# 2InfinityN6eyond/AbsoluteTrack

Measured on AMD Instinct MI355X. Metric: hand-frames/sec, higher is better.
Workload: dtype f32 (backbone products as two fp16 pieces per operand, fp32 accumulation); 1 GPU; 4 fisheye cameras x 2 hands per frame, 2 views per hand, 96x96 crops, known-skeleton path, full hot path (resample+backbone+head+FK) + all-gather of records; frames_per_gpu=1024, src_image=480x636 u8 x 4 cameras, parallelism=frame-shard x1, world=1, backend=none (single process), outputs_finite=True

## Files before the change

### absolutetrack_amd/csrc/conv_w4.hip

```cpp
#include "ut_kernels.h"
#include "ut_conv_dev.h"

namespace ut {
namespace {

constexpr int W4_WPIX = 288;
constexpr int W4_MI = 9;
constexpr int W4_NLOAD = 9;
constexpr int W4_NSTG = 5;
constexpr int W4_DIST = 2;
constexpr int W4_NSET = W4_DIST + 1;
constexpr unsigned W4_HOOB = 0x80000000u;
static_assert(9 % W4_NSET == 0, "the register sets of the weight fragments line up across slices");
constexpr int w4_cap(int pixels, int wi, int hi) { return ((pixels / (wi * hi)) * (hi + 1) * (wi + 1) + 2 * (wi + 2) + 15) / 16 * 16; }

template <int WI, int HI, int SCH, int WPX, bool S2 = false>
__global__ __launch_bounds__(256, 1) void conv_w4_kernel(ConvLaunch p, int tiles_n, int n_tiles) {
  extern __shared__ __attribute__((aligned(16))) char smem[];
  constexpr int MI = W4_MI, PW = WI + 1, PH = HI + 1, HW = WI * HI;
  static_assert(!S2 || (SCH == 32 && WPX == 1), "phase planes: two 16-channel planes per buffer, four 32-channel blocks per tile");
  constexpr int BM = W4_WPIX * WPX;
  constexpr int NCB = 4 / WPX, BN = 32 * NCB;
  constexpr int NG = SCH / 4, NHG = NG / 2;
  constexpr int KS = 9 * SCH / 16;
  constexpr int NBUF = SCH == 32 ? 2 : 3;
  constexpr int AHEAD = NBUF - 1;
  constexpr int RP = 256 / NG;
  constexpr int CAP = w4_cap(BM, WI, HI);
  constexpr int GSTRIDE = CAP * 16;
  constexpr int STAGE = NG * GSTRIDE;
  constexpr int SLOT = NBUF * STAGE;
  constexpr int EPI = SLOT + 16;
  static_assert(BM % HW == 0, "a tile is a whole number of maps: every tile has the same padded layout");
  static_assert(BM * NG == W4_NLOAD * 256 && KS % W4_NSET == 0 && (SCH == 32 || SCH == 16) && (WPX == 1 || WPX == 2), "shape");
  static_assert((NG - 2) * GSTRIDE + (2 * PW + 2) * 16 < 65536, "fragment reads: everything but the lane's base fits the immediate offset");

  const int tid = threadIdx.x;
  const int lane = tid & 63;
  const int wave = __builtin_amdgcn_readfirstlane(tid >> 6);
  const int wm = WPX == 1 ? 0 : wave >> 1;
  const int wco = WPX == 1 ? wave : wave & 1;
  const int fr = lane & 31, fh = lane >> 5;

  const int M = p.n_img * HW;
  const int n_slices = (!S2 && p.k_cin > 0 ? p.k_cin : p.cin) / (S2 ? 16 : SCH);
  const int n_chunks = p.k_pad / 32;

  const __amdgpu_buffer_rsrc_t a_rsrc = __builtin_amdgcn_make_buffer_rsrc(
      const_cast<float*>(p.in), 0, (int)((size_t)M * (S2 ? 4 : 1) * p.cin * sizeof(float)), 0x00020000);
  const __amdgpu_buffer_rsrc_t w_rsrc = __builtin_amdgcn_make_buffer_rsrc(
      const_cast<void*>(p.w_split), 0, (int)((size_t)(p.cout_pad / 32) * n_chunks * 4096), 0x00020000);
  const __amdgpu_buffer_rsrc_t r_rsrc = __builtin_amdgcn_make_buffer_rsrc(
      const_cast<float*>(p.res ? p.res : p.bias), 0, p.res ? (int)((size_t)M * p.cout_store * sizeof(float)) : 0, 0x00020000);
  const __amdgpu_buffer_rsrc_t o_rsrc =
      __builtin_amdgcn_make_buffer_rsrc(p.out, 0, (int)((size_t)M * p.cout_store * sizeof(float)), 0x00020000);
  const __amdgpu_buffer_rsrc_t q_rsrc = __builtin_amdgcn_make_buffer_rsrc(p.tile_counter, 0, 4, 0x00020000);

  float x_scale = 1.f, x_unscale = 1.f;
  if (p.in_max) {
    bool ok, adapted;
    split_act_scale(p.in_max, p.in_obs, p.split_adaptive, x_scale, x_unscale, ok, adapted);
    split_scale_report(ok, adapted, p.status, p.adapt_count);
  }
  const float tot_unscale = p.split_unscale * x_unscale;
  const float floor_v = p.relu ? 0.f : -__builtin_huge_valf();
  const unsigned row_b = (unsigned)p.cout_store * 4u;

  const int grid = gridDim.x;
  int slot = blockIdx.x;
  if ((grid & 7) == 0) slot = (blockIdx.x & 7) * (grid >> 3) + (blockIdx.x >> 3);

  unsigned h_wa[W4_NLOAD], pb[MI];
#pragma unroll
  for (int j = 0; j < W4_NLOAD; ++j) {
    const int k = RP * j + tid / NG, img = k / HW, rem = k - img * HW, y = rem / WI, x = rem - y * WI;
    h_wa[j] = (unsigned)((PW + 1 + img * (PH * PW) + y * PW + x) * 16 + ((tid % NG) >> 1) * GSTRIDE + (tid & 1) * 8);
  }
#pragma unroll
  for (int i = 0; i < MI; ++i) {
    const int k = wm * W4_WPIX + 32 * i + fr, img = k / HW, rem = k - img * HW, y = rem / WI, x = rem - y * WI;
    pb[i] = (unsigned)((img * (PH * PW) + y * PW + x) * 16 + fh * GSTRIDE);
  }
  const unsigned h_step = (unsigned)(RP * p.cin) * 4u;
#define W4_H_BASE(TILE) ((unsigned)((((TILE) / tiles_n) * BM + tid / NG) * p.cin + 4 * (tid % NG)) * 4u)
  unsigned h_in[S2 ? W4_NLOAD : 1], po_a = 0, po_b = 0, pb1[S2 ? MI : 1];
  if constexpr (S2) {
#pragma unroll
    for (int j = 0; j < W4_NLOAD; ++j) {
      const int k = RP * j + tid / NG, img = k / HW, rem = k - img * HW, y = rem / WI, x = rem - y * WI;
      h_in[j] = (unsigned)(((img * 2 * HI + 2 * y) * 2 * WI + 2 * x) * p.cin + 4 * (tid & 3)) * 4u;
    }
    const bool second = (tid & 4) != 0;
    po_a = second ? 0u : (unsigned)((2 * WI + 1) * p.cin) * 4u;
    po_b = second ? (unsigned)(2 * WI * p.cin) * 4u : (unsigned)p.cin * 4u;
#pragma unroll
    for (int i = 0; i < MI; ++i) pb1[i] = pb[i] + (unsigned)STAGE;
  }
#define W4S_BASE(TILE) ((unsigned)(((TILE) / tiles_n) * (BM * 4)) * (unsigned)p.cin * 4u)

  f32x16 acc[MI];
  u32x4 xp[MI][2];
  u32x4 wf[W4_NSET][2];
  float4 stg[S2 ? W4_NLOAD : W4_NSTG];
  const unsigned w_lane = (unsigned)lane * 16u;

#define W4_READ_X(I, PC, S, TAP, BASE)                                                               \
  xp[I][PC] = *reinterpret_cast<const u32x4*>(smem + (BASE)[I] + (unsigned)(((PC) * NHG + (SCH == 32 ? 2 * (S) : 0)) * GSTRIDE + (((TAP) / 3) * PW + (TAP) % 3) * 16));
#define W4_LOAD_W(SET, PL, CH, S, WROW)                                                              \
  {                                                                                                  \
    const unsigned so_ = (WROW) + (unsigned)((wco * n_chunks + (CH)) * 4096 + ((S) * 2 + (PL)) * 1024); \
    wf[SET][PL] = __builtin_bit_cast(u32x4, __builtin_amdgcn_raw_buffer_load_b128(w_rsrc, w_lane, so_, 0)); \
  }
#define W4S_PLANE(Q) ((0x190 >> (Q)) & 1)
#define W4S_TAPP(Q) ((int)((0x414344310ull >> (4 * (Q))) & 15))
#define W4S_TAPO(Q) ((int)((0x715348620ull >> (4 * (Q))) & 15))
#define W4S_BASEOF(Q) ((Q) >= 5 ? pb1 : pb)
#define W4_TAP(Q) (SCH == 32 ? (Q) >> 1 : (Q))
#define W4_CHUNK(SL, Q) (SCH == 32 ? (SL) * 9 + ((Q) >> 1) : ((SL) >> 1) * 9 + (Q))
#define W4_HALF(SL, Q) (SCH == 32 ? (Q) & 1 : (SL) & 1)
#define W4_MFMA(WSET, N)                                                                             \
  {                                                                                                  \
    constexpr int pr_ = (N) / MI, i_ = (N) % MI;                                                     \
    constexpr int wp_ = pr_ == 1 ? 1 : 0, xq_ = pr_ == 0 ? 1 : 0;       \
    acc[i_] = __builtin_amdgcn_mfma_f32_32x32x16_f16(__builtin_bit_cast(f16x8, xp[i_][xq_]),         \
                                                     __builtin_bit_cast(f16x8, wf[WSET][wp_]), acc[i_], 0, 0, 0);  \
  }
#define W4_PIN() { __builtin_amdgcn_sched_barrier(0); asm volatile("" ::: "memory"); __builtin_amdgcn_sched_barrier(0); }
#define W4_ROW_OFF(I, R) ((unsigned)((I) * 32 + 8 * ((R) >> 2) + ((R) & 3)) * row_bs)
#define W4_SPLIT_STORE(V, WA)                                                                        \
  {                                                                                                  \
    unsigned a0_, b0_, a1_, b1_;                                                                     \
    split_pair_scaled((V).x, (V).y, x_scale, a0_, b0_);                                              \
    split_pair_scaled((V).z, (V).w, x_scale, a1_, b1_);                                              \
    *reinterpret_cast<u32x2*>(smem + (WA)) = u32x2{a0_, a1_};                                        \
    *reinterpret_cast<u32x2*>(smem + (WA) + NHG * GSTRIDE) = u32x2{b0_, b1_};                        \
  }

  int tile = slot;
  int next_tile = 0;
  int cur_buf = 0;
  unsigned out_bits = 0;
  const unsigned slot_addr = (unsigned)(unsigned long)(lds_char*)smem + (unsigned)SLOT;

  for (int k = tid; k < NBUF * STAGE / 16; k += 256) *reinterpret_cast<u32x4*>(smem + k * 16) = u32x4{0, 0, 0, 0};
  __syncthreads();
  unsigned h_base = S2 ? 0u : W4_H_BASE(tile);
  unsigned w_row = (unsigned)((tile % tiles_n) * NCB) * (unsigned)n_chunks * 4096u;
  unsigned w_row_next = w_row;
  if constexpr (!S2) {
#pragma unroll
    for (int a = 0; a < AHEAD; ++a)
#pragma unroll
      for (int j = 0; j < W4_NLOAD; ++j) {
        const float4 v = __builtin_bit_cast(float4, __builtin_amdgcn_raw_buffer_load_b128(a_rsrc, h_base + (unsigned)j * h_step, (unsigned)(a * SCH * 4), 0));
        if (a == AHEAD - 1 && KS == 9 && j >= W4_NLOAD - 4) stg[j % W4_NSTG] = v;
        else W4_SPLIT_STORE(v, (unsigned)(a * STAGE) + h_wa[j])
      }
#pragma unroll
    for (int g = 0; g < W4_DIST; ++g) { W4_LOAD_W(g, 0, W4_CHUNK(0, g), W4_HALF(0, g), w_row) W4_LOAD_W(g, 1, W4_CHUNK(0, g), W4_HALF(0, g), w_row) }
  } else {
    const unsigned t0 = W4S_BASE(tile);
#pragma unroll
    for (int j = 0; j < W4_NLOAD; ++j) {
      const float4 v = __builtin_bit_cast(float4, __builtin_amdgcn_raw_buffer_load_b128(a_rsrc, h_in[j] + po_a + t0, 0, 0));
      W4_SPLIT_STORE(v, h_wa[j])
    }
#pragma unroll
    for (int j = 0; j < W4_NLOAD; ++j) {
      const float4 v = __builtin_bit_cast(float4, __builtin_amdgcn_raw_buffer_load_b128(a_rsrc, h_in[j] + po_b + t0, 0, 0));
      if (j == 0) W4_SPLIT_STORE(v, (unsigned)STAGE + h_wa[j])
      else stg[j] = v;
    }
#pragma unroll
    for (int g = 0; g < W4_DIST; ++g) { W4_LOAD_W(g, 0, W4S_TAPO(g), 0, w_row) W4_LOAD_W(g, 1, W4S_TAPO(g), 0, w_row) }
  }
  __syncthreads();
#pragma unroll
  for (int i = 0; i < MI; ++i) {
    W4_READ_X(i, 1, 0, 0, pb)
    if (i < MI - 1) { W4_READ_X(i, 0, 0, 0, pb) }
  }

#define W4_SLOT_BODY(N)                                                                              \
        {                                                                                            \
          if ((N) == 0 && q != KS - 1) { W4_READ_X(MI - 1, 0, W4_HALF(sl, q), W4_TAP(q), rb) }       \
          if ((N) >= 1 && (N) <= 9 && q1 < KS) { W4_READ_X(((N) + 8) % 9, 1, W4_HALF(sl, q1), W4_TAP(q1), rb) } \
          if ((N) >= 1 && (N) <= 9 && q1 == KS) { W4_READ_X(((N) + 8) % 9, 1, 0, 0, nb) }            \
          if ((N) >= 19 && (N) <= 26 && q1 < KS) { W4_READ_X(((N) + 8) % 9, 0, W4_HALF(sl, q1), W4_TAP(q1), rb) } \
          if ((N) >= 19 && (N) <= 26 && q1 == KS) { W4_READ_X(((N) + 8) % 9, 0, 0, 0, nb) }          \
          if (((N) == 10 || (N) == 11) && qd < KS) { W4_LOAD_W(qd % W4_NSET, (N) & 1, W4_CHUNK(sl, qd), W4_HALF(sl, qd), w_row) } \
          if (((N) == 10 || (N) == 11) && qd >= KS) { W4_LOAD_W(qd % W4_NSET, (N) & 1, W4_CHUNK(sl_after, qd - KS), W4_HALF(sl_after, qd - KS), row_after) } \
          if ((N) == 12 && q >= 4 && q < 4 + W4_NLOAD) { const float4 v_ = stg[(q + W4_NSTG - 4) % W4_NSTG]; split_pair_scaled(v_.x, v_.y, x_scale, cv0, cv1); } \
          if ((N) == 13 && q >= 4 && q < 4 + W4_NLOAD) {                                             \
            const float4 v_ = stg[(q + W4_NSTG - 4) % W4_NSTG];                                      \
            unsigned a1_, b1_;                                                                       \
            split_pair_scaled(v_.z, v_.w, x_scale, a1_, b1_);                                        \
            *reinterpret_cast<u32x2*>(smem + wbuf + h_wa[(q + 5) % 9]) = u32x2{cv0, a1_};            \
            *reinterpret_cast<u32x2*>(smem + wbuf + h_wa[(q + 5) % 9] + NHG * GSTRIDE) = u32x2{cv1, b1_}; \
          }                                                                                          \
          if (KS == 9 && (N) == 12 && q < 4) { const float4 v_ = stg[q % W4_NSTG]; split_pair_scaled(v_.x, v_.y, x_scale, cv0, cv1); } \
          if (KS == 9 && (N) == 13 && q < 4) {       \
            const float4 v_ = stg[q % W4_NSTG];                                                      \
            unsigned a1_, b1_;                                                                       \
            split_pair_scaled(v_.z, v_.w, x_scale, a1_, b1_);                                        \
            *reinterpret_cast<u32x2*>(smem + pbuf + h_wa[q + 5]) = u32x2{cv0, a1_};                  \
            *reinterpret_cast<u32x2*>(smem + pbuf + h_wa[q + 5] + NHG * GSTRIDE) = u32x2{cv1, b1_};  \
          }                                                                                          \
          if ((N) == 14 && q < W4_NLOAD)                                                             \
            stg[q % W4_NSTG] = __builtin_bit_cast(float4, __builtin_amdgcn_raw_buffer_load_b128(a_rsrc, h_base + (unsigned)q * h_step, f_soff, 0)); \
          if ((N) == 16 && q == KS / 2 && sl == 0 && tid == 0) *reinterpret_cast<int*>(smem + SLOT) = grid + ticket; \
          W4_PIN();                                                                                  \
          W4_MFMA(ws, N);                                                                            \
          W4_PIN();                                                                                  \
        }
#define W4_SLICE()                                                                                   \
      _Pragma("clang loop unroll(full)") for (int q = 0; q < KS; ++q) {                              \
        const int ws = q % W4_NSET;                                                                  \
        unsigned cv0 = 0, cv1 = 0;      \
         \
        const int q1 = q + 1, qd = q + W4_DIST;                                                      \
        if (q == KS - 1) {                                                                           \
                                       \
          W4_READ_X(MI - 1, 0, W4_HALF(sl, KS - 1), 8, rb)                                           \
          asm volatile("s_waitcnt lgkmcnt(0)" ::: "memory");                                         \
          __builtin_amdgcn_s_barrier();                                                              \
          asm volatile("" ::: "memory");                                                             \
          if (sl == 0) {                                                                             \
            next_tile = slot_read(slot_addr);                                                        \
            w_row_next = (unsigned)((next_tile % tiles_n) * NCB) * (unsigned)n_chunks * 4096u;       \
          }                                                                                          \
        }                                                                                            \
        W4_SLOT_BODY(0) W4_SLOT_BODY(1) W4_SLOT_BODY(2) W4_SLOT_BODY(3) W4_SLOT_BODY(4) W4_SLOT_BODY(5) W4_SLOT_BODY(6) W4_SLOT_BODY(7) W4_SLOT_BODY(8) \
        W4_SLOT_BODY(9) W4_SLOT_BODY(10) W4_SLOT_BODY(11) W4_SLOT_BODY(12) W4_SLOT_BODY(13) W4_SLOT_BODY(14) W4_SLOT_BODY(15) W4_SLOT_BODY(16) W4_SLOT_BODY(17) \
        W4_SLOT_BODY(18) W4_SLOT_BODY(19) W4_SLOT_BODY(20) W4_SLOT_BODY(21) W4_SLOT_BODY(22) W4_SLOT_BODY(23) W4_SLOT_BODY(24) W4_SLOT_BODY(25) W4_SLOT_BODY(26) \
      }

#define W4S_CV_N(Q) ((Q) == 4 ? 3 : (Q) == 8 ? 1 : 2)
#define W4S_CV_J(Q, NN) ((Q) < 4 ? 2 * (Q) + 1 + (NN) : (Q) == 4 ? (NN) : (Q) < 8 ? 2 * (Q) - 7 + (NN) : 0)
#define W4S_CV_DST(Q) (((Q) < 4 || (Q) == 8) ? (unsigned)STAGE : 0u)
#define W4S_LD_N(Q) ((Q) == 0 ? 3 : (Q) == 4 ? 1 : 2)
#define W4S_LD_J(Q, NN) ((Q) == 0 ? (NN) : (Q) < 4 ? 2 * (Q) + 1 + (NN) : (Q) == 4 ? 0 : 2 * (Q) - 9 + (NN))
#define W4S_SLOT_BODY(N)                                                                             \
        {                                                                                            \
          if ((N) == 0) { W4_READ_X(MI - 1, 0, W4S_PLANE(q), W4S_TAPP(q), W4S_BASEOF(q)) }          \
          if ((N) == 9 && (q == 4 || q == 8)) {                                                      \
                                         \
            asm volatile("s_waitcnt lgkmcnt(0)" ::: "memory");                                       \
            __builtin_amdgcn_s_barrier();                                                            \
            asm volatile("" ::: "memory");                                                           \
            if (q == 8 && sl == 0) {                                                                 \
              next_tile = slot_read(slot_addr);                                                      \
              w_row_next = (unsigned)((next_tile % tiles_n) * NCB) * (unsigned)n_chunks * 4096u;     \
            }                                                                                        \
          }                                                                                          \
          if ((N) >= 1 && (N) <= 9 && q != 4 && q != 8) { W4_READ_X(((N) + 8) % 9, 1, W4S_PLANE(q1), W4S_TAPP(q1), W4S_BASEOF(q1)) } \
          if ((N) >= 10 && (N) <= 18 && (q == 4 || q == 8)) { W4_READ_X(((N) + 8) % 9, 1, W4S_PLANE(q1), W4S_TAPP(q1), W4S_BASEOF(q1)) } \
          if ((N) >= 19 && (N) <= 26) { W4_READ_X(((N) + 8) % 9, 0, W4S_PLANE(q1), W4S_TAPP(q1), W4S_BASEOF(q1)) } \
          if (((N) == 10 || (N) == 11) && qd < 9) { W4_LOAD_W(qd % W4_NSET, (N) & 1, (sl >> 1) * 9 + W4S_TAPO(qd), sl & 1, w_row) } \
          if (((N) == 10 || (N) == 11) && qd >= 9) { W4_LOAD_W(qd % W4_NSET, (N) & 1, (sl_after >> 1) * 9 + W4S_TAPO(qd - 9), sl_after & 1, row_after) } \
           \
          if ((N) >= 10 && (N) <= 21 && ((N) - 10) / 4 < W4S_CV_N(q)) {                              \
            const float4 v_ = stg[W4S_CV_J(q, ((N) - 10) / 4) % 9];                                  \
            constexpr int part_ = ((N) - 10) & 3;                                                    \
            if (part_ == 0 || part_ == 2) {                                                          \
              const f16x2 h_ = __builtin_bit_cast(f16x2, __builtin_amdgcn_cvt_pkrtz((part_ ? v_.z : v_.x) * x_scale, (part_ ? v_.w : v_.y) * x_scale)); \
              (part_ ? cvh1 : cvh0) = __builtin_bit_cast(unsigned, h_);                              \
              cvf = (float)h_[0];                                                                    \
            } else {                                                                                 \
              const f16x2 h_ = __builtin_bit_cast(f16x2, part_ == 1 ? cvh0 : cvh1);                  \
              const float ra_ = __builtin_fmaf(part_ == 1 ? v_.x : v_.z, x_scale, -cvf);             \
              const float rb_ = __builtin_fmaf(part_ == 1 ? v_.y : v_.w, x_scale, -(float)h_[1]);    \
              const unsigned p_ = __builtin_bit_cast(unsigned, __builtin_amdgcn_cvt_pkrtz(ra_, rb_)); \
              if (part_ == 1) cvp0 = p_;                                                             \
              else {                                                                                 \
                *reinterpret_cast<u32x2*>(smem + W4S_CV_DST(q) + h_wa[W4S_CV_J(q, ((N) - 10) / 4) % 9]) = u32x2{cvh0, cvh1}; \
                *reinterpret_cast<u32x2*>(smem + W4S_CV_DST(q) + h_wa[W4S_CV_J(q, ((N) - 10) / 4) % 9] + NHG * GSTRIDE) = u32x2{cvp0, p_}; \
              }                                                                                      \
            }                                                                                        \
          }                                                                                          \
          if ((N) >= 22 && (N) <= 24 && (N) - 22 < W4S_LD_N(q))                                      \
            stg[W4S_LD_J(q, (N) - 22) % 9] = __builtin_bit_cast(float4, __builtin_amdgcn_raw_buffer_load_b128(    \
                a_rsrc, h_in[W4S_LD_J(q, (N) - 22) % 9] + (q < 4 ? hb_a : hb_b), f_soff, 0));        \
          if ((N) == 16 && q == 1 && sl == 0 && tid == 0) *reinterpret_cast<int*>(smem + SLOT) = grid + ticket; \
          W4_PIN();                                                                                  \
          W4_MFMA(ws, N);                                                                            \
          W4_PIN();                                                                                  \
        }
#define W4S_SLICE()                                                                                  \
      _Pragma("clang loop unroll(full)") for (int q = 0; q < 9; ++q) {                               \
        const int ws = q % W4_NSET;                                                                  \
        unsigned cvh0 = 0, cvh1 = 0, cvp0 = 0;                       \
        float cvf = 0.f;                                                                             \
        const int q1 = (q + 1) % 9, qd = q + W4_DIST;                                                \
        W4S_SLOT_BODY(0) W4S_SLOT_BODY(1) W4S_SLOT_BODY(2) W4S_SLOT_BODY(3) W4S_SLOT_BODY(4) W4S_SLOT_BODY(5) W4S_SLOT_BODY(6) W4S_SLOT_BODY(7) W4S_SLOT_BODY(8) \
        W4S_SLOT_BODY(9) W4S_SLOT_BODY(10) W4S_SLOT_BODY(11) W4S_SLOT_BODY(12) W4S_SLOT_BODY(13) W4S_SLOT_BODY(14) W4S_SLOT_BODY(15) W4S_SLOT_BODY(16) W4S_SLOT_BODY(17) \
        W4S_SLOT_BODY(18) W4S_SLOT_BODY(19) W4S_SLOT_BODY(20) W4S_SLOT_BODY(21) W4S_SLOT_BODY(22) W4S_SLOT_BODY(23) W4S_SLOT_BODY(24) W4S_SLOT_BODY(25) W4S_SLOT_BODY(26) \
      }

  for (;;) {
    int ticket = 0;
    if (tid == 0) ticket = __builtin_amdgcn_raw_ptr_buffer_atomic_add_i32(1, q_rsrc, 0, 0, 0);
#pragma unroll
    for (int i = 0; i < MI; ++i)
#pragma unroll
      for (int e = 0; e < 16; ++e) acc[i][e] = 0.f;

    const float4 bb4 = *reinterpret_cast<const float4*>(p.bias + (tile % tiles_n) * BN + wco * 32 + 4 * (lane & 7));
    if constexpr (S2) {
      for (int sl = 0; sl < n_slices; ++sl) {
        const bool last_slice = sl == n_slices - 1;
        const unsigned f_soff = last_slice ? 0u : (unsigned)(sl + 1) * 64u;
        const unsigned f_tb = W4S_BASE(last_slice ? next_tile : tile);
        const unsigned hb_a = po_a + f_tb, hb_b = po_b + f_tb;
        const int sl_after = last_slice ? 0 : sl + 1;
        const unsigned row_after = last_slice ? w_row_next : w_row;
        W4S_SLICE()
      }
    } else
    for (int sl = 0; sl < n_slices; ++sl) {
      const bool last_slice = sl == n_slices - 1;
      const int b1 = cur_buf + 1 == NBUF ? 0 : cur_buf + 1, b2 = b1 + 1 == NBUF ? 0 : b1 + 1;
      unsigned rbuf = (unsigned)__builtin_amdgcn_readfirstlane(cur_buf * STAGE), nbuf = (unsigned)__builtin_amdgcn_readfirstlane(b1 * STAGE);
      unsigned wbuf = (unsigned)__builtin_amdgcn_readfirstlane((NBUF == 2 ? b1 : b2) * STAGE), pbuf = nbuf;
      asm volatile("" : "+s"(rbuf), "+s"(nbuf), "+s"(wbuf), "+s"(pbuf));
      const int f_sl = sl + AHEAD < n_slices ? sl + AHEAD : sl + AHEAD - n_slices;
      if (sl + AHEAD == n_slices) h_base = W4_H_BASE(next_tile);
      const unsigned f_soff = (unsigned)f_sl * (SCH * 4);
      const int sl_after = last_slice ? 0 : sl + 1;
      const unsigned row_after = last_slice ? w_row_next : w_row;
      unsigned rb[MI], nb[MI];
#pragma unroll
      for (int i = 0; i < MI; ++i) { rb[i] = pb[i] + rbuf; nb[i] = pb[i] + nbuf; }
      W4_SLICE()
      cur_buf = b1;
    }
    {
      const int tm = tile / tiles_n, tn = tile - tm * tiles_n;
      const bool ragged = tm * BM + BM > M;
      const int ch = tn * BN + wco * 32 + fr;
      const float bb = p.bias[ch];
      const unsigned base = ch < p.cout_store ? (unsigned)((tm * BM + wm * W4_WPIX + 4 * fh) * p.cout_store + ch) * 4u : W4_HOOB;
      const unsigned keep_n = base != W4_HOOB ? 0x7FFFFFFFu : 0u;
      if (!ragged) {
        unsigned row_bs = (unsigned)__builtin_amdgcn_readfirstlane((int)row_b);
        asm volatile("" : "+s"(row_bs));
        const int ch4 = tn * BN + wco * 32 + 4 * (lane & 7);
        const unsigned base4 = ch4 < p.cout_store ? (unsigned)((tm * BM + wm * W4_WPIX + (lane >> 3)) * p.cout_store + ch4) * 4u : W4_HOOB;
        const unsigned keep4 = base4 != W4_HOOB ? 0x7FFFFFFFu : 0u;
        float4 rr[S2 ? 1 : 6][4];
        if constexpr (!S2) {
#pragma unroll
          for (int i = 0; i < 5; ++i)
#pragma unroll
            for (int t = 0; t < 4; ++t)
              rr[i][t] = __builtin_bit_cast(float4, __builtin_amdgcn_raw_buffer_load_b128(r_rsrc, base4, (unsigned)(32 * i + 8 * t) * row_bs, 0));
        }
        char* const ex = smem + EPI + wave * 4096;
#define W4_EX_WRITE(H)                                                                               \
        _Pragma("unroll") for (int r = 0; r < 8; ++r)                                                \
          *reinterpret_cast<float*>(ex + ((H) & 1) * 2048 + (8 * (r >> 2) + 4 * fh + (r & 3)) * 128 + fr * 4) = acc[(H) >> 1][8 * ((H) & 1) + r];
        W4_EX_WRITE(0)
#pragma unroll
        for (int h = 0; h < 2 * MI; ++h) {
          const int i = h >> 1;
          if (!S2 && (h & 1) == 0 && i + 5 < MI) {
#pragma unroll
            for (int t = 0; t < 4; ++t)
              rr[(i + 5) % 6][t] = __builtin_bit_cast(float4, __builtin_amdgcn_raw_buffer_load_b128(r_rsrc, base4, (unsigned)(32 * (i + 5) + 8 * t) * row_bs, 0));
          }
          if (h + 1 < 2 * MI) { W4_EX_WRITE(h + 1) }
#pragma unroll
          for (int t2 = 0; t2 < 2; ++t2) {
            const int t = 2 * (h & 1) + t2;
            const float4 a = *reinterpret_cast<const float4*>(ex + (h & 1) * 2048 + (8 * t2 + (lane >> 3)) * 128 + (lane & 7) * 16);
            const float4 res = S2 ? float4{0.f, 0.f, 0.f, 0.f} : rr[S2 ? 0 : i % 6][t];
            u32x4 o;
            o.x = __float_as_uint(fmaxf(fmaf(a.x, tot_unscale, bb4.x + res.x), floor_v));
            o.y = __float_as_uint(fmaxf(fmaf(a.y, tot_unscale, bb4.y + res.y), floor_v));
            o.z = __float_as_uint(fmaxf(fmaf(a.z, tot_unscale, bb4.z + res.z), floor_v));
            o.w = __float_as_uint(fmaxf(fmaf(a.w, tot_unscale, bb4.w + res.w), floor_v));
            unsigned mk;
            asm volatile("v_max3_u32 %0, %2, %3, %4\n\tv_max_u32 %0, %0, %5\n\tv_and_b32 %0, %0, %6\n\tv_max_u32 %1, %1, %0"
                         : "=&v"(mk), "+v"(out_bits) : "v"(o.x), "v"(o.y), "v"(o.z), "v"(o.w), "v"(keep4));
            __builtin_amdgcn_raw_buffer_store_b128(o, o_rsrc, base4, (unsigned)(32 * i + 8 * t) * row_bs, 0);
          }
        }
#undef W4_EX_WRITE
      } else {
#pragma unroll
        for (int i = 0; i < MI; ++i) {
          float r1[16];
          unsigned off = base + (unsigned)(i * 32) * row_b;
#pragma unroll
          for (int r = 0; r < 16; ++r) {
            r1[r] = __uint_as_float(__builtin_amdgcn_raw_buffer_load_b32(r_rsrc, off, 0, 0));
            off += ((r & 3) == 3 ? 5u : 1u) * row_b;
          }
          off = base + (unsigned)(i * 32) * row_b;
#pragma unroll
          for (int r = 0; r < 16; ++r) {
            const unsigned o = __float_as_uint(fmaxf(fmaf(acc[i][r], tot_unscale, bb + r1[r]), floor_v));
            const int pix = wm * W4_WPIX + i * 32 + 8 * (r >> 2) + 4 * fh + (r & 3);
            out_bits = max(out_bits, o & (tm * BM + pix < M ? keep_n : 0u));
            __builtin_amdgcn_raw_buffer_store_b32(o, o_rsrc, off, 0, 0);
            off += ((r & 3) == 3 ? 5u : 1u) * row_b;
          }
        }
      }
    }
    if ((unsigned)next_tile >= (unsigned)n_tiles) break;
    tile = next_tile;
    w_row = w_row_next;
  }
  if (p.out_max) publish_abs_max(p.out_max, out_bits);
#undef W4_H_BASE
#undef W4_READ_X
#undef W4_LOAD_W
#undef W4_TAP
#undef W4_CHUNK
#undef W4_HALF
#undef W4_MFMA
#undef W4_PIN
#undef W4_ROW_OFF
#undef W4_SPLIT_STORE
#undef W4_SLOT_BODY
#undef W4_SLICE
#undef W4S_PLANE
#undef W4S_TAPP
#undef W4S_TAPO
#undef W4S_BASEOF
#undef W4S_BASE
#undef W4S_CV_N
#undef W4S_CV_J
#undef W4S_CV_DST
#undef W4S_LD_N
#undef W4S_LD_J
#undef W4S_SLOT_BODY
#undef W4S_SLICE
}

template <int WI, int HI, int SCH, int WPX, bool S2 = false>
hipError_t launch_w4_cfg(const ConvLaunch& c, hipStream_t s) {
  constexpr int BM = W4_WPIX * WPX, BN = 128 / WPX;
  const long M = (long)c.n_img * c.Ho * c.Wo;
  const int tiles_m = (int)((M + BM - 1) / BM), tiles_n = c.cout_store / BN;
  const int n_tiles = tiles_m * tiles_n;
  constexpr int lds = (SCH == 32 ? 2 : 3) * (SCH / 4) * w4_cap(BM, WI, HI) * 16 + 16 + 4 * 4096;
  return launch_with_lds<&conv_w4_kernel<WI, HI, SCH, WPX, S2>>(c.device, lds, persistent_grid(c.num_cu, n_tiles), 256, s, c, tiles_n, n_tiles);
}

}

W4Form conv_w4_form(const ConvLaunch& c) {
  const bool common = c.w_split && c.split_unscale > 0.f && c.ksize == 3 && c.pad == 1 && c.cslice == 32 &&
                      c.cin % 32 == 0 && c.cout_pad >= c.cout_store && !c.out_nchw && c.splits == 0 &&
                      c.k_pad == 9 * c.cin && c.tile_counter && c.num_cu > 0 &&
                      offsets_fit_32(c.n_img, c.H, c.W, c.cin) && offsets_fit_32(c.n_img, c.Ho, c.Wo, c.cout_store);
  if (!common) return W4_NONE;
  if (c.stride == 2)
    return c.cin >= 64  && c.cout_store % 128 == 0 && c.H == 2 * c.Ho && c.W == 2 * c.Wo && !c.res &&
           ((c.Wo == 12 && c.Ho == 12) || (c.Wo == 6 && c.Ho == 6)) ? W4_STRIDE2 : W4_NONE;
  if (c.stride != 1 || c.cin < 64 || c.H != c.Ho || c.W != c.Wo) return W4_NONE;
  if (c.k_cin != 0 && (c.k_cin % 32 != 0 || c.k_cin < 64 || c.k_cin > c.cin)) return W4_NONE;
  if (c.cout_store % 128 == 0) return (c.W == 12 && c.H == 12) || (c.W == 6 && c.H == 6) ? W4_TILES128 : W4_NONE;
  return c.cout_store == 64 && c.W == 24 && c.H == 24 ? W4_MAP24 : W4_NONE;
}

hipError_t launch_conv_w4(const ConvLaunch& c, hipStream_t s) {
  const W4Form form = conv_w4_form(c);
  if (form == W4_NONE) return hipErrorInvalidValue;
  if (form == W4_STRIDE2) return c.Wo == 12 ? launch_w4_cfg<12, 12, 32, 1, true>(c, s) : launch_w4_cfg<6, 6, 32, 1, true>(c, s);
  if (form == W4_MAP24) return launch_w4_cfg<24, 24, 16, 2>(c, s);
  return c.W == 12 ? launch_w4_cfg<12, 12, 32, 1>(c, s) : launch_w4_cfg<6, 6, 32, 1>(c, s);
}

}
```

### absolutetrack_amd/csrc/ut_api.hip

```cpp
#include "../../include/umetrack_hip.h"
#include "../../include/umetrack_hip_fit.h"
#include "../../include/umetrack_hip_info.h"
#include "../../include/umetrack_hip_scale.h"
#include "../../include/umetrack_hip_triangulate.h"
#include "../../include/umetrack_hip_views.h"

#include <math.h>
#include <stdio.h>
#include <stdlib.h>
#include <string.h>

#include <cmath>
#include <initializer_list>
#include <mutex>
#include <string>
#include <utility>
#include <vector>

#include "ut_kernels.h"
#include "ut_weights.h"

namespace {

thread_local std::string g_create_error;

struct ConvW : ut::ConvGeom {
  float* w = nullptr;
  float* w_frag = nullptr;
  void* w_split = nullptr;
  float split_unscale = 0.f;
  float wsum_rows = 0.f;
  float bias_max = 0.f;
  float* bias = nullptr;
  int k_cin = 0;
};

struct Block {
  ConvW conv1, conv2, ds;
  bool has_ds = false;
};

struct Regressor {
  Block blocks[2];
  Block blocks_split[2];
  float* w_out = nullptr;
  float* b_out = nullptr;
  int c = 0, d = 0;
};

struct ProfEvent { hipEvent_t a, b; double flops;   int kind = 0;
};

}

constexpr int kDefaultChunk = 4096;
constexpr int kMaxChunk = 7281;

struct ut_context {
  int device = 0;
  int num_cu = 256;
  std::string err;
  std::vector<void*> allocs;
  float* stem_w = nullptr; float* stem_b = nullptr;
  Block bb[12];
  ConvW proj, fus0, fus1, fus2, tmp[3];
  float *skel_w = nullptr, *skel_b = nullptr, *skel_scale = nullptr, *skel_shift = nullptr;
  Regressor reg_k, reg_u;
  int chunk = kDefaultChunk;
  size_t ws_crops = 0;
  float *bufX = nullptr, *bufH = nullptr, *bufY = nullptr, *bufD = nullptr;
  size_t crops_ws_floats = 0;
  float* crops_ws = nullptr;
  size_t wsb_crops = 0;
  float *bufL2 = nullptr, *bufP = nullptr, *bufQ = nullptr, *bufBH = nullptr, *bufBD = nullptr;
  size_t ws_samples = 0;
  ut::HeadBuffers hb{};
  size_t ws_skel = 0;
  int slots_cap = 0, slots_used = 0;
  float *mem = nullptr, *prev_ext = nullptr;
  unsigned* counters = nullptr;
  int counter_next = 0;
  unsigned* calib = nullptr;
  unsigned* adapt_count = nullptr;
  int scale_mode = UT_SPLIT_SCALE_CALIBRATED;
  bool calibrated = false;
  bool head_calibrated = false;
  bool calibrating = false;
  unsigned word_gen = 0;
  bool block_fusion = true;
  int resident_weights = 1;
  bool call_split = false;
  int* status = nullptr;
  int* status_host = nullptr;
  int* slot_seen = nullptr;
  int check_mode = UT_CHECK_SYNC;
  int lanes = 1;
  hipStream_t lane_stream[2] = {nullptr, nullptr};
  hipEvent_t ev_fork = nullptr, ev_join[2] = {nullptr, nullptr};
  int conv_arith = UT_CONV_FP32;
  bool latency_mode = false;
  float* splitk_ws = nullptr;
  size_t splitk_floats = 0;
  float* zero_bias = nullptr;
  bool profiling = false;
  std::vector<ProfEvent> prof;
};

namespace {

int fail(ut_handle h, int code, const char* what, hipError_t e = hipSuccess) {
  char buf[512];
  if (e != hipSuccess) snprintf(buf, sizeof buf, "%s: %s", what, hipGetErrorString(e));
  else snprintf(buf, sizeof buf, "%s", what);
  if (h) h->err = buf; else g_create_error = buf;
  return code;
}

#define HIPCHK(h, x)                                            \
  do {                                                          \
    hipError_t e_ = (x);                                        \
    if (e_ != hipSuccess) return fail(h, UT_E_HIP, #x, e_);     \
  } while (0)

struct DeviceScope {
  int prev = -1;
  bool switched = false;
  hipError_t err = hipSuccess;
  explicit DeviceScope(int dev) {
    if (dev < 0) return;
    err = hipGetDevice(&prev);
    if (err == hipSuccess && prev != dev) {
      err = hipSetDevice(dev);
      switched = err == hipSuccess;
    }
  }
  ~DeviceScope() { if (switched) (void)hipSetDevice(prev); }
  DeviceScope(const DeviceScope&) = delete;
  DeviceScope& operator=(const DeviceScope&) = delete;
};
#define ON_DEVICE_IF(h)                                        \
  DeviceScope scope_((h) ? (h)->device : -1);                  \
  if ((h) && scope_.err != hipSuccess) return fail(h, UT_E_HIP, "hipSetDevice", scope_.err)
#define ON_DEVICE_OF(h)                 \
  DeviceScope scope_((h)->device);      \
  if (scope_.err != hipSuccess) return fail(h, UT_E_HIP, "hipSetDevice", scope_.err)

struct DevStatus { int* dev = nullptr; int* host = nullptr; };
std::mutex g_status_mutex;
DevStatus g_status[64];

int stateless_status(int* device_out, DevStatus* out) {
  int dev = 0;
  hipError_t e = hipGetDevice(&dev);
  if (e != hipSuccess) return fail(nullptr, UT_E_HIP, "hipGetDevice", e);
  if (dev < 0 || dev >= 64) return fail(nullptr, UT_E_INVALID, "device index beyond 63");
  std::lock_guard<std::mutex> lock(g_status_mutex);
  DevStatus& st = g_status[dev];
  if (!st.dev) {
    void *d = nullptr, *hst = nullptr;
    if ((e = hipMalloc(&d, 2 * sizeof(int))) != hipSuccess) return fail(nullptr, UT_E_HIP, "hipMalloc", e);
    if ((e = hipHostMalloc(&hst, 2 * sizeof(int), hipHostMallocDefault)) != hipSuccess) {
      (void)hipFree(d);
      return fail(nullptr, UT_E_HIP, "hipHostMalloc", e);
    }
    if ((e = hipMemset(d, 0, 2 * sizeof(int))) != hipSuccess) return fail(nullptr, UT_E_HIP, "hipMemset", e);
    st.dev = (int*)d; st.host = (int*)hst;
  }
  *device_out = dev;
  *out = st;
  return UT_OK;
}

const char* status_message(int bits) {
  if (bits & ut::UT_SPLIT_RANGE)
    return "range check: an activation entering a split-fp16 convolution is an infinity or a NaN, or lies beyond the calibrated range "
           "of its layer (32 x the calibration maximum; ut_calibrate_split with representative crops, UT_SPLIT_SCALE_DYNAMIC or "
           "UT_SPLIT_SCALE_CALIBRATED_ADAPTIVE)";
  if (bits & ut::UT_BAD_SRC_INDEX) return "index check: src_index outside [0, n_src_images)";
  if (bits & ut::UT_BAD_SAMPLE_RANGE) return "index check: sample_range rows must select 1 or 2 crops inside [0, n_crops]";
  if (bits & ut::UT_BAD_MEMORY_IDX) return "index check: memory_idx outside [0, n_slots)";
  if (bits & ut::UT_DUP_MEMORY_IDX) return "index check: memory_idx names one temporal slot twice";
  if (bits & ut::UT_BAD_HAND_IDX) return "index check: hand_idx must be 0 (left) or 1 (right)";
  return "index check: failed";
}

int check_status(ut_handle h, int* dev, int* host, hipStream_t s, const char* what) {
  HIPCHK(h, hipMemcpyAsync(host, dev, 2 * sizeof(int), hipMemcpyDeviceToHost, s));
  HIPCHK(h, hipStreamSynchronize(s));
  const int sticky = host[0];
  if (sticky) HIPCHK(h, hipMemsetAsync(dev, 0, sizeof(int), s));
  if (sticky & ut::UT_STATUS_ERRORS) {
    char buf[256];
    snprintf(buf, sizeof buf, "%s: %s", what, status_message(sticky));
    return fail(h, UT_E_INVALID, buf);
  }
  return UT_OK;
}

int upload_bytes(ut_handle h, const void* host, size_t bytes, void** dev) {
  void* d = nullptr;
  HIPCHK(h, hipMalloc(&d, bytes));
  h->allocs.push_back(d);
  HIPCHK(h, hipMemcpy(d, host, bytes, hipMemcpyHostToDevice));
  *dev = d;
  return UT_OK;
}

int upload(ut_handle h, const std::vector<float>& host, float** dev) {
  return upload_bytes(h, host.data(), host.size() * sizeof(float), (void**)dev);
}

int upload_conv(ut_handle h, ConvW& cw, const ut::PackedConv& pc) {
  static_cast<ut::ConvGeom&>(cw) = pc;
  cw.split_unscale = pc.split_unscale; cw.wsum_rows = pc.wsum_rows; cw.bias_max = pc.bias_max;
  int rc = upload(h, pc.wp, &cw.w);
  if (!rc && !pc.wfrag.empty()) rc = upload(h, pc.wfrag, &cw.w_frag);
  if (!rc && !pc.planes.empty()) rc = upload_bytes(h, pc.planes.data(), pc.planes.size() * sizeof(uint16_t), &cw.w_split);
  return rc ? rc : upload(h, pc.bp, &cw.bias);
}

int upload_block(ut_handle h, Block& b, const ut::FoldedBlock& fb, bool pw_ds = false) {
  int rc;
  const int cs = ut::round_up(fb.conv1.cout, 4);
  if ((rc = upload_conv(h, b.conv1, ut::pack_conv_host(fb.conv1, 3, fb.stride, cs)))) return rc;
  if ((rc = upload_conv(h, b.conv2, ut::pack_conv_host(fb.conv2, 3, 1, cs)))) return rc;
  b.has_ds = fb.has_ds;
  if (fb.has_ds && (rc = upload_conv(h, b.ds, ut::pack_conv_host(fb.ds, 1, fb.stride, cs, pw_ds)))) return rc;
  return UT_OK;
}

int upload_regressor(ut_handle h, Regressor& r, const ut::FoldedRegressor& fr) {
  r.c = fr.c; r.d = fr.d;
  int rc;
  for (int i = 0; i < 2; ++i)
    if ((rc = upload_block(h, r.blocks[i], fr.blocks[i])) || (rc = upload_block(h, r.blocks_split[i], fr.wide[i]))) return rc;
  for (int i = 0; i < 2; ++i) {
    r.blocks_split[i].conv1.k_cin = ut::round_up(fr.blocks[i].conv1.cin, 32);
    r.blocks_split[i].conv2.k_cin = ut::round_up(fr.blocks[i].conv2.cin, 32);
  }
  if ((rc = upload(h, fr.w_out, &r.w_out))) return rc;
  return upload(h, fr.b_out, &r.b_out);
}

int dev_alloc(ut_handle h, float** p, size_t n_floats) {
  void* d = nullptr;
  HIPCHK(h, hipMalloc(&d, n_floats * sizeof(float)));
  h->allocs.push_back(d);
  *p = (float*)d;
  return UT_OK;
}

void dev_free(ut_handle h, void* p) {
  if (!p) return;
  for (size_t i = 0; i < h->allocs.size(); ++i)
    if (h->allocs[i] == p) { h->allocs.erase(h->allocs.begin() + i); break; }
  (void)hipFree(p);
}

int regrow(ut_handle h, size_t* cap, size_t n, std::initializer_list<std::pair<float**, size_t>> bufs) {
  if (n <= *cap) return UT_OK;
  HIPCHK(h, hipDeviceSynchronize());
  for (auto& b : bufs) { dev_free(h, *b.first); *b.first = nullptr; }
  *cap = 0;
  int rc;
  for (auto& b : bufs)
    if ((rc = dev_alloc(h, b.first, n * b.second))) return rc;
  *cap = n;
  return UT_OK;
}

int ensure_backbone_ws(ut_handle h, int crops) {
  const size_t big = 48 * 48 * 32, small = 24 * 24 * 64;
  return regrow(h, &h->ws_crops, crops, {{&h->bufX, big}, {&h->bufH, big}, {&h->bufY, big}, {&h->bufD, small}});
}

constexpr int PHASE_B_MAX = 8192;

int ensure_phase_b_ws(ut_handle h, int crops) {
  const size_t l2 = 24 * 24 * 64, l3 = 12 * 12 * 128;
  return regrow(h, &h->wsb_crops, crops, {{&h->bufL2, l2}, {&h->bufP, l3}, {&h->bufQ, l3}, {&h->bufBH, l3}, {&h->bufBD, l3}});
}

int ensure_head_ws(ut_handle h, int samples, int n_skel) {
  ut::HeadBuffers& b = h->hb;
  const size_t r = 36 * ut::kRegSplitCh;
  int rc = regrow(h, &h->ws_samples, samples, {{&b.cat144, 36 * 144}, {&b.f108, 36 * 108}, {&b.f72a, 36 * 72}, {&b.f72b, 36 * 72},
                                                {&b.fused, 36 * 72}, {&b.t92a, 36 * 92}, {&b.t92b, 36 * 92}, {&b.regin, r},
                                                {&b.rega, r}, {&b.regb, r}});
  return rc ? rc : regrow(h, &h->ws_skel, n_skel, {{&b.skel, 36 * 4}});
}

int ensure_slots(ut_handle h, int slots, hipStream_t s) {
  if (slots <= h->slots_cap) return UT_OK;
  int cap = h->slots_cap ? h->slots_cap : 2;
  while (cap < slots) cap *= 2;
  float *nm = nullptr, *ne = nullptr, *seen = nullptr;
  int rc;
  if ((rc = dev_alloc(h, &nm, (size_t)cap * 36 * 18)) || (rc = dev_alloc(h, &ne, (size_t)cap * 16)) ||
      (rc = dev_alloc(h, &seen, (size_t)cap)))
    return rc;
  HIPCHK(h, hipMemsetAsync(nm, 0, (size_t)cap * 36 * 18 * sizeof(float), s));
  HIPCHK(h, hipMemsetAsync(ne, 0, (size_t)cap * 16 * sizeof(float), s));
  if (h->slots_cap) {
    HIPCHK(h, hipMemcpyAsync(nm, h->mem, (size_t)h->slots_cap * 36 * 18 * sizeof(float), hipMemcpyDeviceToDevice, s));
    HIPCHK(h, hipMemcpyAsync(ne, h->prev_ext, (size_t)h->slots_cap * 16 * sizeof(float), hipMemcpyDeviceToDevice, s));
    HIPCHK(h, hipStreamSynchronize(s));
    dev_free(h, h->mem);
    dev_free(h, h->prev_ext);
    dev_free(h, h->slot_seen);
  }
  h->mem = nm; h->prev_ext = ne; h->slot_seen = (int*)seen; h->slots_cap = cap;
  return UT_OK;
}

constexpr int kMaxCounters = 4096;
constexpr int kScaleTensors = 33;
static_assert(kScaleTensors < 63, "the adaptation counter is the last of the 64 words at ut_context::calib");
constexpr int kCalibHeadroom = 4;

int begin_call(ut_handle h, hipStream_t s) {
  h->counter_next = 0;
  ++h->word_gen;
  HIPCHK(h, ut::launch_zero_words(h->counters, 2 * kMaxCounters, s));
  return UT_OK;
}

int lease_words(ut_handle h, hipStream_t s, int n, bool* zeroed = nullptr) {
  const bool full = h->counter_next + n > kMaxCounters;
  if (zeroed) *zeroed = full;
  return full ? begin_call(h, s) : UT_OK;
}
int take_word(ut_handle h) { return h->counter_next++; }

struct ScaleRef { const unsigned* word = nullptr; const unsigned* obs = nullptr; int adaptive = 0; unsigned* adapt_count = nullptr; };
ScaleRef scale_for(ut_handle h, int tid, const unsigned* producer_word) {
  ScaleRef r;
  if (!h->call_split || h->latency_mode || tid < 0 || tid >= kScaleTensors) return r;
  if (h->calibrating || h->scale_mode == UT_SPLIT_SCALE_DYNAMIC) r.word = producer_word;
  else { r.word = h->calib + tid; r.obs = producer_word; }
  if (!h->calibrating && h->scale_mode == UT_SPLIT_SCALE_CALIBRATED_ADAPTIVE && r.obs) { r.adaptive = 1; r.adapt_count = h->adapt_count; }
  return r;
}
template <class Launch>
void set_scale(Launch& l, const ScaleRef& sr, int* status) {
  l.in_max = sr.word; l.in_obs = sr.obs; l.split_adaptive = sr.adaptive; l.adapt_count = sr.adapt_count; l.status = status;
}
template <class Launch>
int bracket_launch(ut_handle h, hipStream_t s, int in_tid, const unsigned* in_max, double flops, int kind, const char* what,
                   Launch launch) {
  if (h->calibrating && in_max && in_tid >= 0 && in_tid < kScaleTensors) HIPCHK(h, ut::launch_merge_max(h->calib + in_tid, in_max, s));
  ProfEvent pe{nullptr, nullptr, flops, kind};
  if (h->profiling) {
    HIPCHK(h, hipEventCreateWithFlags(&pe.a, hipEventDisableSystemFence));
    HIPCHK(h, hipEventCreateWithFlags(&pe.b, hipEventDisableSystemFence));
    HIPCHK(h, hipEventRecord(pe.a, s));
  }
  const hipError_t e = launch();
  if (e != hipSuccess) return fail(h, UT_E_HIP, what, e);
  if (h->profiling) {
    HIPCHK(h, hipEventRecord(pe.b, s));
    h->prof.push_back(pe);
  }
  return UT_OK;
}

int run_conv(ut_handle h, const ConvW& cw, const float* in, const float* res, float* out, int n_img, int H, int W,
             bool relu, bool nchw, hipStream_t s, const unsigned* in_max = nullptr, unsigned** out_max = nullptr, int in_tid = -1) {
  if (out_max) *out_max = nullptr;
  ut::ConvLaunch c{};
  c.in = in; c.w = cw.w; c.bias = cw.bias; c.res = res; c.out = out;
  c.n_img = n_img; c.H = H; c.W = W; c.cin = cw.cin_pad;
  c.Ho = (H + 2 * cw.pad - cw.ksize) / cw.stride + 1;
  c.Wo = (W + 2 * cw.pad - cw.ksize) / cw.stride + 1;
  c.cout_store = cw.cout_store; c.cout_pad = cw.cout_pad;
  c.k_total = cw.k_total; c.k_pad = cw.k_pad; c.cslice = cw.cslice;
  c.k_cin = h->block_fusion && cw.k_cin < cw.cin_pad ? cw.k_cin : 0;
  c.ksize = cw.ksize; c.stride = cw.stride; c.pad = cw.pad;
  c.relu = relu; c.out_nchw = nchw;
  c.device = h->device; c.num_cu = h->num_cu; c.no_resident = ut::kResidentKinds[h->resident_weights];
  bool zeroed = false;
  int rc = lease_words(h, s, 1, &zeroed);
  if (rc) return rc;
  if (zeroed) in_max = nullptr;
  const int word = take_word(h);
  c.tile_counter = h->counters + word;
  int splits = 1;
  if (h->latency_mode && !nchw && cw.cout_store % 4 == 0) {
    const long m = (long)n_img * c.Ho * c.Wo;
    const long tiles64 = ((m + 63) / 64) * ((cw.cout_store + 63) / 64);
    const int chunks = cw.k_pad / 32;
    for (int sp = 2; sp <= chunks / 6; ++sp)
      if (chunks % sp == 0 && tiles64 * sp <= (long)h->num_cu && (size_t)sp * m * cw.cout_store <= h->splitk_floats) splits = sp;
  }
  if (h->latency_mode) c.splits = 1;
  if (splits > 1) {
    ut::ConvLaunch part = c;
    part.bias = h->zero_bias; part.res = nullptr; part.relu = 0; part.out = h->splitk_ws; part.splits = splits;
    HIPCHK(h, ut::launch_conv_igemm(part, s));
    HIPCHK(h, ut::launch_splitk_finish(h->splitk_ws, splits, n_img * c.Ho * c.Wo, cw.cout_store, cw.bias, res, out,
                                       relu ? 1 : 0, s));
    return UT_OK;
  }
  const ScaleRef sr = scale_for(h, in_tid, in_max);
  c.w_split = sr.word ? cw.w_split : nullptr;
  c.split_unscale = cw.split_unscale;
  set_scale(c, sr, h->status);
  const ut::ConvKernel kernel = ut::choose_conv(c);
  const int kind = c.w_split && kernel != ut::CONV_IGEMM ? 1 : 0;
  if (kind) {
    c.out_max = h->counters + kMaxCounters + word;
    if (out_max) *out_max = c.out_max;
  }
  return bracket_launch(h, s, kind ? in_tid : -1, in_max, cw.flops_per_pixel * (double)n_img * c.Ho * c.Wo, kind,
                        ut::kConvKernelName[kernel], [&] { return ut::launch_conv_on(kernel, c, s); });
}

int run_pw(ut_handle h, std::initializer_list<const ConvW*> layers, std::initializer_list<bool> relus, const float* in, float* out,
           int n_img, int H, int W, bool nchw, hipStream_t s, bool* done) {
  *done = false;
  if (!h->block_fusion || h->latency_mode) return UT_OK;
  ut::PwLaunch c{};
  double flops = 0;
  const ConvW& first = **layers.begin();
  c.in = in; c.out = out; c.n_img = n_img; c.H = H; c.W = W; c.cin = first.cin_pad; c.stride = first.stride;
  c.Ho = (H - 1) / first.stride + 1; c.Wo = (W - 1) / first.stride + 1;
  c.out_nchw = nchw; c.num_cu = h->num_cu;
  auto relu = relus.begin();
  for (const ConvW* cw : layers) {
    if (cw->ksize != 1 || cw->pad != 0 || !cw->w_frag || (c.n_layers > 0 && cw->stride != 1)) return UT_OK;
    c.layer[c.n_layers++] = ut::PwLayer{cw->w_frag, cw->bias, cw->k_pad, cw->cout_store, cw->cout_pad, *relu++ ? 1 : 0};
    c.cout_store = cw->cout_store;
    flops += cw->flops_per_pixel * (double)n_img * c.Ho * c.Wo;
  }
  if (!ut::conv_pw_applicable(c)) return UT_OK;
  *done = true;
  return bracket_launch(h, s, -1, nullptr, flops, 0, "launch_conv_pw", [&] { return ut::launch_conv_pw(c, s); });
}

int run_block(ut_handle h, const Block& b, const float* x, float* tmp, float* dsbuf, float* y, int n_img, int H,
              int W, hipStream_t s, const unsigned* x_max = nullptr, unsigned** y_max = nullptr, int x_tid = -1, int mid_tid = -1) {
  int rc;
  if (y_max) *y_max = nullptr;
  bool zeroed = false;
  if ((rc = lease_words(h, s, 8, &zeroed))) return rc;
  if (zeroed) x_max = nullptr;
  const ScaleRef xs = scale_for(h, x_tid, x_max);
  if (h->block_fusion && xs.word && !b.has_ds && b.conv1.w_split && b.conv2.w_split && b.conv1.stride == 1 &&
      b.conv1.cin_pad == 32 && b.conv1.cout_store == 32 && b.conv2.cout_store == 32) {
    ut::BlockLaunch bl{};
    bl.in = x; bl.out = y; bl.w1_split = b.conv1.w_split; bl.w2_split = b.conv2.w_split;
    bl.unscale_w1 = b.conv1.split_unscale; bl.unscale_w2 = b.conv2.split_unscale;
    bl.bias1 = b.conv1.bias; bl.bias2 = b.conv2.bias;
    bl.wsum1 = b.conv1.wsum_rows; bl.bmax1 = b.conv1.bias_max;
    set_scale(bl, xs, h->status);
    bl.n_img = n_img; bl.H = H; bl.W = W; bl.device = h->device; bl.num_cu = h->num_cu;
    bl.tile_counter = h->counters + h->counter_next;
    if (ut::conv_block32_applicable(bl)) {
      bl.out_max = h->counters + kMaxCounters + take_word(h);
      const double flops = (b.conv1.flops_per_pixel + b.conv2.flops_per_pixel) * (double)n_img * H * W;
      if ((rc = bracket_launch(h, s, x_tid, x_max, flops, 1, "conv_block32", [&] { return ut::launch_conv_block32(bl, s); })))
        return rc;
      if (y_max) *y_max = bl.out_max;
      return UT_OK;
    }
  }
  if (h->block_fusion && xs.word && b.has_ds && b.conv1.w_split && b.ds.w_split && b.conv2.w_split &&
      b.conv1.stride == 2 && b.conv1.cin_pad == 32 && b.conv1.cout_store == 64 && b.ds.cout_store == 64 && dsbuf) {
    ut::Stride2Launch sl{};
    sl.in = x; sl.out1 = tmp; sl.out2 = dsbuf; sl.w1_split = b.conv1.w_split; sl.wd_split = b.ds.w_split;
    sl.unscale1 = b.conv1.split_unscale; sl.unscale_d = b.ds.split_unscale;
    sl.bias1 = b.conv1.bias; sl.bias_d = b.ds.bias;
    set_scale(sl, xs, h->status);
    sl.n_img = n_img; sl.H = H; sl.W = W; sl.device = h->device; sl.num_cu = h->num_cu;
    if (ut::conv_c32s2_applicable(sl)) {
      sl.out1_max = h->counters + kMaxCounters + take_word(h);
      const double flops = (b.conv1.flops_per_pixel + b.ds.flops_per_pixel) * (double)n_img * (H / 2) * (W / 2);
      if ((rc = bracket_launch(h, s, x_tid, x_max, flops, 1, "conv_c32s2", [&] { return ut::launch_conv_c32s2(sl, s); })))
        return rc;
      return run_conv(h, b.conv2, tmp, dsbuf, y, n_img, H / 2, W / 2, true, false, s, sl.out1_max, y_max, mid_tid);
    }
  }
  unsigned* tmp_max = nullptr;
  if ((rc = run_conv(h, b.conv1, x, nullptr, tmp, n_img, H, W, true, false, s, x_max, &tmp_max, x_tid))) return rc;
  const int Ho = (H + 2 - 3) / b.conv1.stride + 1, Wo = (W + 2 - 3) / b.conv1.stride + 1;
  const float* res = x;
  if (b.has_ds) {
    bool streamed = false;
    if ((rc = run_pw(h, {&b.ds}, {false}, x, dsbuf, n_img, H, W, false, s, &streamed))) return rc;
    if (!streamed && (rc = run_conv(h, b.ds, x, nullptr, dsbuf, n_img, H, W, false, false, s))) return rc;
    res = dsbuf;
  }
  return run_conv(h, b.conv2, tmp, res, y, n_img, Ho, Wo, true, false, s, tmp_max, y_max, mid_tid);
}

void prof_clear(ut_handle h) {
  for (auto& pe : h->prof) { (void)hipEventDestroy(pe.a); (void)hipEventDestroy(pe.b); }
  h->prof.clear();
}

int prof_reduce(ut_handle h, hipStream_t s, double ms[2], int64_t launches[2], double flops[2]) {
  h->profiling = false;
  HIPCHK(h, hipStreamSynchronize(s));
  for (int k = 0; k < 2; ++k) { ms[k] = 0; launches[k] = 0; flops[k] = 0; }
  for (auto& pe : h->prof) {
    float t = 0;
    HIPCHK(h, hipEventElapsedTime(&t, pe.a, pe.b));
    const int k = pe.kind ? 1 : 0;
    ms[k] += t; flops[k] += pe.flops; launches[k] += 1;
  }
  prof_clear(h);
  return UT_OK;
}

}

extern "C" {

size_t ut_weight_blob_floats(void) { return UT_WEIGHT_BLOB_FLOATS; }

const char* ut_last_error(ut_handle h) { return h ? h->err.c_str() : g_create_error.c_str(); }

int ut_canonical_backbone_weights(const float* blob, size_t n_floats, float* out, size_t out_floats, size_t* n_out) {
  if (!blob || !n_out) return fail(nullptr, UT_E_INVALID, "ut_canonical_backbone_weights: null argument");
  if (n_floats != UT_WEIGHT_BLOB_FLOATS) return fail(nullptr, UT_E_WEIGHTS, "ut_canonical_backbone_weights: weight blob has the wrong length");
  ut::FoldedNetwork net;
  if (!ut::fold_network(blob, n_floats, net)) return fail(nullptr, UT_E_WEIGHTS, "weight blob length does not match the architecture");
  const ut::FoldedBackbone& fbb = net.backbone;
  std::vector<const ut::Folded*> all = {&fbb.stem};
  for (const ut::FoldedBlock& b : fbb.fb) {
    all.push_back(&b.conv1); all.push_back(&b.conv2);
    if (b.has_ds) all.push_back(&b.ds);
  }
  all.push_back(&fbb.proj);
  size_t n = 0;
  for (const ut::Folded* f : all) n += f->w.size() + f->b.size();
  *n_out = n;
  if (!out) return UT_OK;
  if (out_floats < n) return fail(nullptr, UT_E_INVALID, "ut_canonical_backbone_weights: output too small");
  for (const ut::Folded* f : all) {
    memcpy(out, f->w.data(), f->w.size() * sizeof(float)); out += f->w.size();
    memcpy(out, f->b.data(), f->b.size() * sizeof(float)); out += f->b.size();
  }
  return UT_OK;
}

int ut_create(int device, const float* blob, size_t n_floats, ut_handle* out) {
  if (!blob || !out) return fail(nullptr, UT_E_INVALID, "ut_create: null argument");
  if (n_floats != UT_WEIGHT_BLOB_FLOATS) return fail(nullptr, UT_E_WEIGHTS, "ut_create: weight blob has the wrong length");
  ut::FoldedNetwork net;
  if (!ut::fold_network(blob, n_floats, net)) return fail(nullptr, UT_E_WEIGHTS, "weight blob length does not match the architecture");
  DeviceScope scope(device);
  if (scope.err != hipSuccess) return fail(nullptr, UT_E_HIP, "hipSetDevice", scope.err);
  ut_handle h = new ut_context();
  h->device = device;
  {
    int cus = 0;
    if (hipDeviceGetAttribute(&cus, hipDeviceAttributeMultiprocessorCount, device) == hipSuccess && cus > 0) h->num_cu = cus;
  }
  int rc = UT_OK;
  do {
    { float* cnt = nullptr; if ((rc = dev_alloc(h, &cnt, 2 * kMaxCounters + 64))) break; h->counters = (unsigned*)cnt;
      h->calib = h->counters + 2 * kMaxCounters;
      h->adapt_count = h->calib + 63;
      hipError_t e1 = hipMemset(h->calib, 0, 64 * sizeof(unsigned));
      if (e1 != hipSuccess) { rc = fail(h, UT_E_HIP, "calibration words", e1); break; } }
    { float* st = nullptr; if ((rc = dev_alloc(h, &st, 2))) break; h->status = (int*)st;
      hipError_t e2 = hipMemset(h->status, 0, 2 * sizeof(int));
      if (e2 == hipSuccess) e2 = hipHostMalloc((void**)&h->status_host, 2 * sizeof(int), hipHostMallocDefault);
      if (e2 != hipSuccess) { rc = fail(h, UT_E_HIP, "status words", e2); break; } }
    const ut::FoldedBackbone& fbb = net.backbone;
    if ((rc = upload(h, fbb.stem.w, &h->stem_w)) || (rc = upload(h, fbb.stem.b, &h->stem_b))) break;
    for (int b = 0; b < 12 && !rc; ++b) rc = upload_block(h, h->bb[b], fbb.fb[b], b == 10);
    if (rc) break;
    if ((rc = upload_conv(h, h->proj, ut::pack_conv_host(fbb.proj, 1, 1, 72, true)))) break;
    if ((rc = upload_conv(h, h->fus0, ut::pack_conv_host(net.fusion[0], 1, 1, 108, true))) ||
        (rc = upload_conv(h, h->fus1, ut::pack_conv_host(net.fusion[1], 1, 1, 72, true))) ||
        (rc = upload_conv(h, h->fus2, ut::pack_conv_host(net.fusion[2], 1, 1, 72, true)))) break;
    for (int i = 0; i < 3 && !rc; ++i) rc = upload_conv(h, h->tmp[i], ut::pack_conv_host(net.temporal[i], 1, 1, 92, true));
    if (rc) break;
    if ((rc = upload(h, net.skel_w, &h->skel_w)) || (rc = upload(h, net.skel_b, &h->skel_b)) ||
        (rc = upload(h, net.skel_scale, &h->skel_scale)) || (rc = upload(h, net.skel_shift, &h->skel_shift))) break;
    if ((rc = upload_regressor(h, h->reg_k, net.reg_k))) break;
    rc = upload_regressor(h, h->reg_u, net.reg_u);
  } while (0);
  if (rc) {
    g_create_error = h->err;
    ut_destroy(h);
    return rc;
  }
  *out = h;
  return UT_OK;
}

int ut_destroy(ut_handle h) {
  if (!h) return UT_OK;
  DeviceScope scope(h->device);
  (void)hipDeviceSynchronize();
  for (void* p : h->allocs) (void)hipFree(p);
  if (h->status_host) (void)hipHostFree(h->status_host);
  for (int i = 0; i < 2; ++i) {
    if (h->lane_stream[i]) (void)hipStreamDestroy(h->lane_stream[i]);
    if (h->ev_join[i]) (void)hipEventDestroy(h->ev_join[i]);
  }
  if (h->ev_fork) (void)hipEventDestroy(h->ev_fork);
  prof_clear(h);
  delete h;
  return UT_OK;
}

int ut_set_backbone_chunk(ut_handle h, int crops_per_pass) {
  if (!h || crops_per_pass < 0) return fail(h, UT_E_INVALID, "ut_set_backbone_chunk: bad argument");
  if (crops_per_pass > kMaxChunk) return fail(h, UT_E_INVALID, "ut_set_backbone_chunk: at most 7281 crops per pass (32-bit offsets)");
  h->chunk = crops_per_pass == 0 ? kDefaultChunk : crops_per_pass;
  return UT_OK;
}

int ut_reserve(ut_handle h, int max_crops, int max_samples, int max_slots) {
  if (!h) return UT_E_INVALID;
  ON_DEVICE_OF(h);
  int rc;
  int c = max_crops < h->chunk ? max_crops : h->chunk;
  if (c > 0 && (rc = ensure_backbone_ws(h, c))) return rc;
  int cb = max_crops < PHASE_B_MAX ? max_crops : PHASE_B_MAX;
  if (cb > 0 && (rc = ensure_phase_b_ws(h, cb))) return rc;
  if (max_samples > 0 && (rc = ensure_head_ws(h, max_samples, max_samples))) return rc;
  if (max_slots > 0 && (rc = ensure_slots(h, max_slots, 0))) return rc;
  if (max_crops > 0 && (rc = regrow(h, &h->crops_ws_floats, (size_t)max_crops * 96 * 96, {{&h->crops_ws, 1}}))) return rc;
  return UT_OK;
}

int ut_warp_crops(ut_handle h, const uint8_t* src, int n_src_images, int src_h, int src_w, const double* cam_params,
                  const double* crop_params, const int32_t* src_index, int n_crops, int remap_mode, float* out,
                  void* stream) {
  if (n_crops == 0) return UT_OK;
  if (!src || !cam_params || !crop_params || !src_index || !out || n_crops < 0 || src_h <= 0 || src_w <= 0 ||
      n_src_images <= 0 || (remap_mode != UT_REMAP_CV2_FIXED && remap_mode != UT_REMAP_FLOAT))
    return fail(h, UT_E_INVALID, "ut_warp_crops: bad argument");
  hipStream_t s = (hipStream_t)stream;
  int *st_dev = nullptr, *st_host = nullptr, mode = UT_CHECK_SYNC, dev = 0;
  if (h) { st_dev = h->status; st_host = h->status_host; mode = h->check_mode; dev = h->device; }
  else {
    DevStatus st;
    int rc = stateless_status(&dev, &st);
    if (rc) return rc;
    st_dev = st.dev; st_host = st.host;
  }
  DeviceScope scope(dev);
  if (scope.err != hipSuccess) return fail(h, UT_E_HIP, "hipSetDevice", scope.err);
  HIPCHK(h, ut::launch_warp(src, n_src_images, src_h, src_w, cam_params, crop_params, src_index, n_crops, remap_mode,
                            out, nullptr, st_dev, s));
  return mode == UT_CHECK_SYNC ? check_status(h, st_dev, st_host, s, "ut_warp_crops") : UT_OK;
}

extern "C" int ut_warp_map(const double* cam_params, const double* crop_params, const int32_t* src_index, int n_src_images,
                           int n_crops, float* out_map, void* stream) {
  if (n_crops == 0) return UT_OK;
  if (!cam_params || !crop_params || !src_index || !out_map || n_crops < 0 || n_src_images <= 0)
    return fail(nullptr, UT_E_INVALID, "ut_warp_map: bad argument");
  HIPCHK(nullptr, ut::launch_warp_map(cam_params, crop_params, src_index, n_src_images, n_crops, out_map, (hipStream_t)stream));
  return UT_OK;
}

static int run_stem(ut_handle h, const float* crops, const uint8_t* crops_u8, float* out, int n, hipStream_t st,
                    unsigned** out_max) {
  *out_max = nullptr;
  if (h->call_split && !h->latency_mode) {
    const int rc = lease_words(h, st, 1);
    if (rc) return rc;
    *out_max = h->counters + kMaxCounters + take_word(h);
  }
  if (crops_u8) HIPCHK(h, ut::launch_stem_u8(crops_u8, h->stem_w, h->stem_b, out, n, *out_max, st));
  else HIPCHK(h, ut::launch_stem(crops, h->stem_w, h->stem_b, out, n, *out_max, st));
  return UT_OK;
}

static int backbone_pass(ut_handle h, const float* crops, const uint8_t* crops_u8, float* feat, int c0, int n, int off,
                         int chunk, hipStream_t s) {
  int rc;
  const size_t a48 = (size_t)off * 48 * 48 * 32, a24 = (size_t)off * 24 * 24 * 64, a12 = (size_t)off * 12 * 12 * 128;
  if ((rc = lease_words(h, s, 256))) return rc;
  unsigned* l2_max = nullptr;
  const unsigned l2_gen = h->word_gen;
  for (int done = 0; done < n; done += chunk) {
    const int m = n - done < chunk ? n - done : chunk;
    const size_t first = (size_t)(c0 + done) * 96 * 96;
    unsigned* xm = nullptr;
    if ((rc = run_stem(h, crops ? crops + first : nullptr, crops_u8 ? crops_u8 + first : nullptr, h->bufX + a48, m, s, &xm))) return rc;
    float *x = h->bufX + a48, *y = h->bufY + a48;
    int hw = 48;
    for (int b = 0; b < 5; ++b) {
      float* dst = b == 4 ? h->bufL2 + a24 + (size_t)done * 24 * 24 * 64 : y;
      if ((rc = run_block(h, h->bb[b], x, h->bufH + a48, h->bufD + a24, dst, m, hw, hw, s, xm, &xm, 2 * b, 2 * b + 1))) return rc;
      hw = (hw + 2 - 3) / h->bb[b].conv1.stride + 1;
      float* t = x; x = y; y = t;
    }
    if (done == 0) l2_max = xm;
    else if (l2_max && xm) HIPCHK(h, ut::launch_merge_max(l2_max, xm, s));
    else l2_max = nullptr;
  }
  const float* x = h->bufL2 + a24;
  float *y = h->bufP + a12, *other = h->bufQ + a12;
  int hw = 24;
  unsigned* xm = l2_gen == h->word_gen ? l2_max : nullptr;
  for (int b = 5; b < 12; ++b) {
    if ((rc = run_block(h, h->bb[b], x, h->bufBH + a12, h->bufBD + a12, y, n, hw, hw, s, xm, &xm, 2 * b, 2 * b + 1))) return rc;
    hw = (hw + 2 - 3) / h->bb[b].conv1.stride + 1;
    x = y;
    float* t = y; y = other; other = t;
  }
  bool streamed = false;
  if ((rc = run_pw(h, {&h->proj}, {false}, x, feat + (size_t)c0 * 72 * 36, n, 6, 6, true, s, &streamed)) || streamed) return rc;
  return run_conv(h, h->proj, x, nullptr, feat + (size_t)c0 * 72 * 36, n, 6, 6, false, true, s);
}

static int run_backbone(ut_handle h, const float* crops, const uint8_t* crops_u8, int n_crops, float* feat, hipStream_t s) {
  int rc;
  const int chunk = n_crops < h->chunk ? n_crops : h->chunk;
  if ((rc = ensure_backbone_ws(h, chunk))) return rc;
  const int pass_b = n_crops < PHASE_B_MAX ? n_crops : PHASE_B_MAX;
  if ((rc = ensure_phase_b_ws(h, pass_b))) return rc;
  if ((rc = begin_call(h, s))) return rc;
  h->call_split = h->conv_arith == UT_CONV_SPLIT_F16_ALWAYS || (h->conv_arith == UT_CONV_SPLIT_F16 && n_crops >= 2 * h->num_cu);
  if (h->lanes == 2 && !h->profiling && n_crops <= chunk && n_crops <= pass_b && n_crops >= 1024) {
    if (!h->lane_stream[0]) {
      for (int i = 0; i < 2; ++i) {
        HIPCHK(h, hipStreamCreateWithFlags(&h->lane_stream[i], hipStreamNonBlocking));
        HIPCHK(h, hipEventCreateWithFlags(&h->ev_join[i], hipEventDisableTiming));
      }
      HIPCHK(h, hipEventCreateWithFlags(&h->ev_fork, hipEventDisableTiming));
    }
    HIPCHK(h, hipEventRecord(h->ev_fork, s));
    const int n0 = n_crops / 2;
    for (int i = 0; i < 2; ++i) {
      const int off = i ? n0 : 0, n = i ? n_crops - n0 : n0;
      HIPCHK(h, hipStreamWaitEvent(h->lane_stream[i], h->ev_fork, 0));
      if ((rc = backbone_pass(h, crops, crops_u8, feat, off, n, off, chunk, h->lane_stream[i]))) return rc;
      HIPCHK(h, hipEventRecord(h->ev_join[i], h->lane_stream[i]));
    }
    for (int i = 0; i < 2; ++i) HIPCHK(h, hipStreamWaitEvent(s, h->ev_join[i], 0));
    return UT_OK;
  }
  for (int base = 0; base < n_crops; base += pass_b) {
    const int nb = n_crops - base < pass_b ? n_crops - base : pass_b;
    if ((rc = backbone_pass(h, crops, crops_u8, feat, base, nb, 0, chunk, s))) return rc;
  }
  return UT_OK;
}

static int run_head(ut_handle h, const ut::HeadArgs& a, const float* skel, int n_skel, int mode, float* out_pose, float* out_raw,
                    hipStream_t s);

static int calibrate_head(ut_handle h, const float* feat, int n_crops, hipStream_t s) {
  const int S = n_crops / 2;
  int rc = ensure_head_ws(h, S, 1);
  if (rc) return rc;
  const size_t nf = (size_t)2 * S * 25 + 132 + (size_t)S * (648 + 16 + 60 + 64);
  const size_t off_i64 = (nf * 4 + 7) / 8 * 8, off_i32 = off_i64 + (size_t)4 * S * 8, off_u8 = off_i32 + (size_t)S * 4, total = off_u8 + S;
  std::vector<char> host(total, 0);
  float* f = reinterpret_cast<float*>(host.data());
  for (int c = 0; c < 2 * S; ++c) {
    float* k = f + (size_t)c * 9;
    k[0] = k[4] = 130.f; k[2] = k[5] = 47.5f; k[8] = 1.f;
    float* x = f + (size_t)2 * S * 9 + (size_t)c * 16;
    x[0] = x[5] = x[10] = x[15] = 1.f;
    if (c & 1) x[3] = 0.06f;
  }
  long long* i64 = reinterpret_cast<long long*>(host.data() + off_i64);
  for (int k = 0; k < S; ++k) { i64[2 * k] = 2 * k; i64[2 * k + 1] = 2 * k + 2; i64[2 * S + k] = k; i64[3 * S + k] = k & 1; }
  void* dv = nullptr;
  HIPCHK(h, hipMalloc(&dv, total));
  hipError_t e = hipMemcpyAsync(dv, host.data(), total, hipMemcpyHostToDevice, s);
  if (e == hipSuccess) e = hipStreamSynchronize(s);
  if (e != hipSuccess) { (void)hipFree(dv); return fail(h, UT_E_HIP, "calibration descriptors", e); }
  char* d = static_cast<char*>(dv);
  float* df = reinterpret_cast<float*>(d);
  ut::HeadArgs a{};
  a.feat = feat; a.intrinsics = df; a.extrinsics = df + (size_t)2 * S * 9;
  const float* skel = df + (size_t)2 * S * 25;
  a.mem = df + (size_t)2 * S * 25 + 132; a.prev_ext = a.mem + (size_t)S * 648;
  float* pose = a.prev_ext + (size_t)S * 16;
  float* raw = pose + (size_t)S * 60;
  a.sample_range = reinterpret_cast<const int64_t*>(d + off_i64); a.memory_idx = a.sample_range + 2 * S; a.hand_idx = a.memory_idx + S;
  a.slot_seen = reinterpret_cast<int*>(d + off_i32); a.use_memory = reinterpret_cast<const uint8_t*>(d + off_u8);
  a.n_samples = S; a.n_crops = 2 * S; a.n_slots = S; a.status = h->status; a.call_error_mask = 0;
  rc = begin_call(h, s);
  for (int mode = 0; mode < 2 && !rc; ++mode) rc = run_head(h, a, skel, 1, mode == 0 ? UT_MODE_KNOWN_SKELETON : UT_MODE_UNKNOWN_SKELETON, pose, raw, s);
  (void)hipStreamSynchronize(s);
  (void)hipFree(dv);
  return rc;
}

static int calibrate_split(ut_handle h, const float* crops, int n, hipStream_t s) {
  struct PinnedModes {
    ut_handle h;
    const int conv_arith, lanes;
    const bool profiling, block_fusion, latency_mode;
    explicit PinnedModes(ut_handle hh)
        : h(hh), conv_arith(hh->conv_arith), lanes(hh->lanes), profiling(hh->profiling), block_fusion(hh->block_fusion),
          latency_mode(hh->latency_mode) {
      h->conv_arith = UT_CONV_SPLIT_F16_ALWAYS; h->lanes = 1; h->profiling = false; h->latency_mode = false; h->calibrating = true;
    }
    ~PinnedModes() {
      h->conv_arith = conv_arith; h->lanes = lanes; h->profiling = profiling; h->block_fusion = block_fusion;
      h->latency_mode = latency_mode; h->calibrating = false;
    }
  };
  float* feat = nullptr;
  int rc = dev_alloc(h, &feat, (size_t)n * 72 * 36);
  if (rc) return rc;
  rc = [&]() -> int {
    PinnedModes pinned(h);
    int saved[2] = {0, 0}, r;
    HIPCHK(h, hipStreamSynchronize(s));
    HIPCHK(h, hipMemcpy(saved, h->status, sizeof saved, hipMemcpyDeviceToHost));
    h->calibrated = h->head_calibrated = false;
    HIPCHK(h, ut::launch_zero_words(h->calib, 64, s));
    for (int form = 0; form < 2; ++form) {
      h->block_fusion = form == 0;
      if ((r = run_backbone(h, crops, nullptr, n, feat, s))) return r;
    }
    const bool with_head = n >= 2;
    if (with_head && (r = calibrate_head(h, feat, n, s))) return r;
    HIPCHK(h, ut::launch_raise_words(h->calib, kScaleTensors, kCalibHeadroom, s));
    HIPCHK(h, hipStreamSynchronize(s));
    HIPCHK(h, hipMemcpy(h->status, saved, sizeof saved, hipMemcpyHostToDevice));
    h->calibrated = true;
    h->head_calibrated = with_head;
    return UT_OK;
  }();
  (void)hipStreamSynchronize(s);
  dev_free(h, feat);
  return rc;
}

constexpr int kBuiltinCalibCrops = 64;

static int calibrate_builtin(ut_handle h) {
  float* crops = nullptr;
  int rc = dev_alloc(h, &crops, (size_t)kBuiltinCalibCrops * 96 * 96);
  if (rc) return rc;
  hipError_t e = ut::launch_calibration_crops(crops, kBuiltinCalibCrops, 0);
  rc = e != hipSuccess ? fail(h, UT_E_HIP, "launch_calibration_crops", e) : calibrate_split(h, crops, kBuiltinCalibCrops, 0);
  (void)hipDeviceSynchronize();
  dev_free(h, crops);
  return rc;
}

int ut_calibrate_split(ut_handle h, const float* crops, int n_crops, void* stream) {
  if (!h) return UT_E_INVALID;
  if (n_crops < 0 || (n_crops > 0 && !crops)) return fail(h, UT_E_INVALID, "ut_calibrate_split: bad argument");
  ON_DEVICE_OF(h);
  return n_crops == 0 ? calibrate_builtin(h) : calibrate_split(h, crops, n_crops, (hipStream_t)stream);
}

int ut_set_split_scale(ut_handle h, int mode) {
  if (!h || (mode != UT_SPLIT_SCALE_CALIBRATED && mode != UT_SPLIT_SCALE_DYNAMIC && mode != UT_SPLIT_SCALE_CALIBRATED_ADAPTIVE))
    return fail(h, UT_E_INVALID, "ut_set_split_scale: bad argument");
  ON_DEVICE_OF(h);
  h->scale_mode = mode;
  if (mode != UT_SPLIT_SCALE_DYNAMIC && h->conv_arith != UT_CONV_FP32 && !h->calibrated) return calibrate_builtin(h);
  return UT_OK;
}

int ut_get_split_adaptations(ut_handle h, uint32_t* out, int reset, void* stream) {
  if (!h || !out) return fail(h, UT_E_INVALID, "ut_get_split_adaptations: null argument");
  ON_DEVICE_OF(h);
  hipStream_t s = (hipStream_t)stream;
  unsigned n = 0;
  HIPCHK(h, hipMemcpyAsync(&n, h->adapt_count, sizeof n, hipMemcpyDeviceToHost, s));
  HIPCHK(h, hipStreamSynchronize(s));
  *out = n;
  if (reset) {
    HIPCHK(h, ut::launch_zero_words(h->adapt_count, 1, s));
    HIPCHK(h, hipStreamSynchronize(s));
  }
  return UT_OK;
}

int ut_get_split_calibration(ut_handle h, float* out33) {
  if (!h || !out33) return fail(h, UT_E_INVALID, "ut_get_split_calibration: null argument");
  ON_DEVICE_OF(h);
  HIPCHK(h, hipDeviceSynchronize());
  HIPCHK(h, hipMemcpy(out33, h->calib, kScaleTensors * sizeof(float), hipMemcpyDeviceToHost));
  return h->calibrated ? UT_OK : 1;
}

int ut_backbone(ut_handle h, const float* crops, int n_crops, float* feat, void* stream) {
  if (!h) return UT_E_INVALID;
  if (n_crops == 0) return UT_OK;
  if (!crops || !feat || n_crops < 0) return fail(h, UT_E_INVALID, "ut_backbone: bad argument");
  ON_DEVICE_OF(h);
  return run_backbone(h, crops, nullptr, n_crops, feat, (hipStream_t)stream);
}

int ut_warp_backbone(ut_handle h, const uint8_t* src, int n_src_images, int src_h, int src_w, const double* cam_params,
                     const double* crop_params, const int32_t* src_index, int n_crops, int remap_mode, float* feat,
                     void* stream) {
  if (!h) return UT_E_INVALID;
  if (n_crops == 0) return UT_OK;
  if (!src || !cam_params || !crop_params || !src_index || !feat || n_crops < 0 || src_h <= 0 || src_w <= 0 ||
      n_src_images <= 0 || (remap_mode != UT_REMAP_CV2_FIXED && remap_mode != UT_REMAP_FLOAT))
    return fail(h, UT_E_INVALID, "ut_warp_backbone: bad argument");
  ON_DEVICE_OF(h);
  hipStream_t s = (hipStream_t)stream;
  const bool u8 = remap_mode == UT_REMAP_CV2_FIXED;
  int rc = regrow(h, &h->crops_ws_floats, (size_t)n_crops * 96 * 96 / (u8 ? sizeof(float) : 1), {{&h->crops_ws, 1}});
  if (rc) return rc;
  HIPCHK(h, ut::launch_warp(src, n_src_images, src_h, src_w, cam_params, crop_params, src_index, n_crops, remap_mode,
                            u8 ? nullptr : h->crops_ws, u8 ? (uint8_t*)h->crops_ws : nullptr, h->status, s));
  if (h->check_mode == UT_CHECK_SYNC && (rc = check_status(h, h->status, h->status_host, s, "ut_warp_backbone"))) return rc;
  return run_backbone(h, u8 ? nullptr : h->crops_ws, u8 ? (const uint8_t*)h->crops_ws : nullptr, n_crops, feat, s);
}

static int run_head(ut_handle h, const ut::HeadArgs& a, const float* skel, int n_skel, int mode, float* out_pose, float* out_raw,
                    hipStream_t s) {
  int rc;
  const ut::HeadBuffers& b = h->hb;
  const int S = a.n_samples;
  h->call_split = false;
  HIPCHK(h, ut::launch_ftl_in(a, b, h->block_fusion, s));
  bool chained = false;
  if ((rc = run_pw(h, {&h->fus0, &h->fus1, &h->fus2}, {true, true, false}, b.cat144, b.f72b, S, 6, 6, false, s, &chained))) return rc;
  if (!chained) {
    if ((rc = run_conv(h, h->fus0, b.cat144, nullptr, b.f108, S, 6, 6, true, false, s))) return rc;
    if ((rc = run_conv(h, h->fus1, b.f108, nullptr, b.f72a, S, 6, 6, true, false, s))) return rc;
    if ((rc = run_conv(h, h->fus2, b.f72a, nullptr, b.f72b, S, 6, 6, false, false, s))) return rc;
  }
  HIPCHK(h, ut::launch_ftl_out_temporal_in(a, b, s));
  if ((rc = run_pw(h, {&h->tmp[0], &h->tmp[1], &h->tmp[2]}, {true, true, false}, b.t92a, b.t92b, S, 6, 6, false, s, &chained))) return rc;
  if (!chained) {
    if ((rc = run_conv(h, h->tmp[0], b.t92a, nullptr, b.t92b, S, 6, 6, true, false, s))) return rc;
    if ((rc = run_conv(h, h->tmp[1], b.t92b, nullptr, b.t92a, S, 6, 6, true, false, s))) return rc;
    if ((rc = run_conv(h, h->tmp[2], b.t92a, nullptr, b.t92b, S, 6, 6, false, false, s))) return rc;
  }
  const Regressor& reg = mode == UT_MODE_KNOWN_SKELETON ? h->reg_k : h->reg_u;
  if (mode == UT_MODE_KNOWN_SKELETON)
    HIPCHK(h, ut::launch_skeleton(skel, h->skel_w, h->skel_b, h->skel_scale, h->skel_shift, b.skel, n_skel, s));
  const bool head_split = !h->latency_mode && (h->calibrating || h->scale_mode == UT_SPLIT_SCALE_DYNAMIC || h->head_calibrated) &&
                          (h->conv_arith == UT_CONV_SPLIT_F16_ALWAYS || (h->conv_arith == UT_CONV_SPLIT_F16 && S >= 4 * h->num_cu));
  const int stride = head_split ? ut::kRegSplitCh : reg.c;
  const int tid0 = mode == UT_MODE_KNOWN_SKELETON ? 25 : 29;
  unsigned* in_word = nullptr;
  if (head_split) {
    if ((rc = lease_words(h, s, 16))) return rc;
    in_word = h->counters + kMaxCounters + take_word(h);
  }
  HIPCHK(h, ut::launch_temporal_out(a, b.t92b, b.skel, n_skel, b.regin, reg.c, stride, in_word, s));
  h->call_split = head_split;
  const Block* blocks = head_split ? reg.blocks_split : reg.blocks;
  unsigned* mid_word = nullptr;
  rc = run_block(h, blocks[0], b.regin, b.rega, nullptr, b.regb, S, 6, 6, s, in_word, &mid_word, head_split ? tid0 : -1, head_split ? tid0 + 1 : -1);
  if (!rc) rc = run_block(h, blocks[1], b.regb, b.rega, nullptr, b.regin, S, 6, 6, s, mid_word, nullptr, head_split ? tid0 + 2 : -1, head_split ? tid0 + 3 : -1);
  h->call_split = false;
  if (rc) return rc;
  HIPCHK(h, ut::launch_pool_decode(a, b.regin, reg.c, stride, reg.w_out, reg.b_out, reg.d, out_pose, out_raw, b.rega, s));
  return UT_OK;
}

int ut_fuse_temporal_regress(ut_handle h, const float* feat, const float* intrinsics, const float* extrinsics,
                             const int64_t* sample_range, const int64_t* memory_idx, const uint8_t* use_memory,
                             const int64_t* hand_idx, int n_crops, int n_samples, int n_slots, int all_multiview,
                             const float* skel, int n_skel, int mode, float* out_pose, float* out_raw, void* stream) {
  if (!h) return UT_E_INVALID;
  if (n_samples == 0) return UT_OK;
  if (!feat || !intrinsics || !extrinsics || !sample_range || !memory_idx || !use_memory || !hand_idx || !out_pose ||
      n_samples < 0 || n_crops < n_samples || n_crops > 2 * n_samples || n_slots <= 0)
    return fail(h, UT_E_INVALID, "ut_fuse_temporal_regress: bad argument");
  if (mode == UT_MODE_KNOWN_SKELETON) {
    if (!skel || (n_skel != 1 && n_skel != n_samples))
      return fail(h, UT_E_INVALID, "ut_fuse_temporal_regress: skeleton must have 1 or n_samples entries");
  } else if (mode == UT_MODE_UNKNOWN_SKELETON) {
    if (!all_multiview)
      return fail(h, UT_E_UNSUPPORTED, "Unsupported: found single-view samples when calibration scale");
    n_skel = 0;
  } else {
    return fail(h, UT_E_INVALID, "ut_fuse_temporal_regress: unknown mode");
  }
  ON_DEVICE_OF(h);
  hipStream_t s = (hipStream_t)stream;
  int rc;
  if ((rc = ensure_head_ws(h, n_samples, n_skel))) return rc;
  if ((rc = ensure_slots(h, n_slots, s))) return rc;
  if ((rc = begin_call(h, s))) return rc;
  h->call_split = false;
  ut::HeadArgs a{};
  a.feat = feat; a.intrinsics = intrinsics; a.extrinsics = extrinsics; a.sample_range = sample_range;
  a.memory_idx = memory_idx; a.use_memory = use_memory; a.hand_idx = hand_idx; a.n_samples = n_samples;
  a.n_crops = n_crops; a.n_slots = n_slots;
  a.mem = h->mem; a.prev_ext = h->prev_ext;
  a.status = h->status; a.slot_seen = h->slot_seen;
  a.call_error_mask = mode == UT_MODE_UNKNOWN_SKELETON ? ut::UT_SINGLE_VIEW : 0;
  HIPCHK(h, ut::launch_zero_words(h->status + 1, 1, s));
  HIPCHK(h, ut::launch_zero_words(h->slot_seen, (size_t)n_slots, s));
  HIPCHK(h, ut::launch_validate_desc(a, s));
  if (h->check_mode == UT_CHECK_SYNC) {
    if ((rc = check_status(h, h->status, h->status_host, s, "ut_fuse_temporal_regress"))) return rc;
    if (h->status_host[1] & a.call_error_mask)
      return fail(h, UT_E_UNSUPPORTED, "Unsupported: found single-view samples when calibration scale");
  }
  if (n_slots > h->slots_used) h->slots_used = n_slots;
  return run_head(h, a, skel, n_skel, mode, out_pose, out_raw, s);
}

int ut_reset_memory(ut_handle h) {
  if (!h) return UT_E_INVALID;
  ON_DEVICE_OF(h);
  HIPCHK(h, hipDeviceSynchronize());
  if (h->slots_cap) {
    HIPCHK(h, hipMemset(h->mem, 0, (size_t)h->slots_cap * 36 * 18 * sizeof(float)));
    HIPCHK(h, hipMemset(h->prev_ext, 0, (size_t)h->slots_cap * 16 * sizeof(float)));
  }
  h->slots_used = 0;
  return UT_OK;
}

int ut_get_memory(ut_handle h, float* mem, float* prev_ext, int max_slots, void* stream) {
  if (!h) return UT_E_INVALID;
  ON_DEVICE_OF(h);
  int n = h->slots_used < max_slots ? h->slots_used : max_slots;
  if (n > 0) {
    if (!mem || !prev_ext) return fail(h, UT_E_INVALID, "ut_get_memory: null output");
    HIPCHK(h, ut::launch_mem_export(h->mem, mem, n, (hipStream_t)stream));
    HIPCHK(h, hipMemcpyAsync(prev_ext, h->prev_ext, (size_t)n * 16 * sizeof(float), hipMemcpyDeviceToDevice,
                             (hipStream_t)stream));
  }
  return h->slots_used;
}

int ut_fk(ut_handle h, const float* hand_model, int n_models, const float* joint_angles, int ja_stride,
          const float* wrist_xf, int xf_stride, const int64_t* mirror, float t_scale, int n, float* out, void* stream) {
  if (n == 0) return UT_OK;
  if (!hand_model || !joint_angles || !wrist_xf || !out || n < 0 || (n_models != 1 && n_models != n) ||
      ja_stride < 22 || xf_stride < 16)
    return fail(h, UT_E_INVALID, "ut_fk: bad argument");
  ON_DEVICE_IF(h);
  HIPCHK(h, ut::launch_fk(hand_model, n_models, joint_angles, ja_stride, wrist_xf, xf_stride, mirror, t_scale, n, out,
                          (hipStream_t)stream));
  return UT_OK;
}

namespace {
int fail_as(ut_handle h, const char* who, const char* what) {
  char msg[256];
  snprintf(msg, sizeof msg, "%s: %s", who, what);
  return fail(h, UT_E_INVALID, msg);
}

int fit_pose_args(ut_handle h, const char* who, const float* hand_model, int n_models, const float* targets, int target_stride,
                  const float* init_angles, int init_ja_stride, const float* init_wrist_xf, int init_xf_stride, float t_scale,
                  int max_iters, int n, const float* joint_angles, int ja_stride, const float* wrist_xf, int xf_stride,
                  bool with_targets = true) {
  if (!hand_model || (with_targets && !targets) || !joint_angles || !wrist_xf || n < 0 || (n_models != 1 && n_models != n))
    return fail_as(h, who, "bad argument");
  if (!with_targets && (!init_angles || !init_wrist_xf))
    return fail_as(h, who, "init_angles and init_wrist_xf are required: there is no cold start");
  if ((init_angles == nullptr) != (init_wrist_xf == nullptr))
    return fail_as(h, who, "init_angles and init_wrist_xf must both be given or both be NULL");
  if ((with_targets && target_stride < 63) || ja_stride < 22 || xf_stride < 12 || (init_angles && (init_ja_stride < 22 || init_xf_stride < 12)))
    return fail_as(h, who, "a stride is below 63 (targets) / 22 (angles) / 12 (wrist)");
  if (max_iters < 1 || max_iters > 256) return fail_as(h, who, "max_iters must be in 1..256");
  if (!(t_scale > 0.f) || !(t_scale <= 3.0e38f)) return fail_as(h, who, "t_scale must be positive and finite");
  return UT_OK;
}
}

int ut_fit_pose(ut_handle h, const float* hand_model, int n_models, const float* targets, int target_stride,
                const float* weights, const float* limits, const float* init_angles, int init_ja_stride,
                const float* init_wrist_xf, int init_xf_stride, const int64_t* mirror, float t_scale, int max_iters, int n,
                float* joint_angles, int ja_stride, float* wrist_xf, int xf_stride, float* info, void* stream) {
  if (n == 0) return UT_OK;
  const int rc = fit_pose_args(h, "ut_fit_pose", hand_model, n_models, targets, target_stride, init_angles, init_ja_stride,
                               init_wrist_xf, init_xf_stride, t_scale, max_iters, n, joint_angles, ja_stride, wrist_xf, xf_stride);
  if (rc) return rc;
  ON_DEVICE_IF(h);
  const ut::FitArgs a{{hand_model, n_models, targets, target_stride, limits, init_angles, init_ja_stride, init_wrist_xf,
                       init_xf_stride, mirror, t_scale, max_iters, n, joint_angles, ja_stride, wrist_xf, xf_stride},
                      weights, info};
  HIPCHK(h, ut::launch_fit_pose(a, (hipStream_t)stream));
  return UT_OK;
}

int ut_fit_pose_info(ut_handle h, const float* hand_model, int n_models, const float* targets, int target_stride,
                     const float* sqrt_info, const float* limits, const float* init_angles, int init_ja_stride,
                     const float* init_wrist_xf, int init_xf_stride, const int64_t* mirror, float t_scale, int max_iters, int n,
                     float* joint_angles, int ja_stride, float* wrist_xf, int xf_stride, float* info, void* stream) {
  if (n == 0) return UT_OK;
  if (!sqrt_info) return fail(h, UT_E_INVALID, "ut_fit_pose_info: bad argument");
  const int rc = fit_pose_args(h, "ut_fit_pose_info", hand_model, n_models, targets, target_stride, init_angles, init_ja_stride,
                               init_wrist_xf, init_xf_stride, t_scale, max_iters, n, joint_angles, ja_stride, wrist_xf, xf_stride);
  if (rc) return rc;
  ON_DEVICE_IF(h);
  const ut::FitInfoArgs a{{hand_model, n_models, targets, target_stride, limits, init_angles, init_ja_stride, init_wrist_xf,
                           init_xf_stride, mirror, t_scale, max_iters, n, joint_angles, ja_stride, wrist_xf, xf_stride},
                          sqrt_info, info};
  HIPCHK(h, ut::launch_fit_pose_info(a, (hipStream_t)stream));
  return UT_OK;
}

static_assert(UT_SCALE_FREE == ut::FITS_MODE_FREE && UT_SCALE_FIXED == ut::FITS_MODE_FIXED && UT_SCALE_MIN == ut::FITS_SCALE_MIN &&
              UT_SCALE_MAX == ut::FITS_SCALE_MAX && UT_SCALE_INFO_LAMBDA == ut::FITS_SCALE_INFO_LAMBDA &&
              UT_FITS_CONVERGED == ut::FITS_CONVERGED && UT_FITS_AT_MAX_ITERS == ut::FITS_AT_MAX_ITERS &&
              UT_FITS_REFUSED == ut::FITS_REFUSED && UT_FITS_AT_BOUND == ut::FITS_AT_BOUND, "umetrack_hip_scale.h and ut_kernels.h");

int ut_fit_pose_scale(ut_handle h, const float* hand_model, int n_models, const float* targets, int target_stride,
                      const float* weights, const float* limits, const float* init_scale, int scale_mode,
                      const float* init_angles, int init_ja_stride, const float* init_wrist_xf, int init_xf_stride,
                      const int64_t* mirror, float t_scale, int max_iters, int n, float* joint_angles, int ja_stride,
                      float* wrist_xf, int xf_stride, float* scale, float* info, void* stream) {
  if (n == 0) return UT_OK;
  if (!scale) return fail(h, UT_E_INVALID, "ut_fit_pose_scale: bad argument");
  if (scale_mode != UT_SCALE_FREE && scale_mode != UT_SCALE_FIXED)
    return fail(h, UT_E_INVALID, "ut_fit_pose_scale: scale_mode must be UT_SCALE_FREE or UT_SCALE_FIXED");
  const int rc = fit_pose_args(h, "ut_fit_pose_scale", hand_model, n_models, targets, target_stride, init_angles, init_ja_stride,
                               init_wrist_xf, init_xf_stride, t_scale, max_iters, n, joint_angles, ja_stride, wrist_xf, xf_stride);
  if (rc) return rc;
  ON_DEVICE_IF(h);
  const ut::FitScaleArgs a{{hand_model, n_models, targets, target_stride, limits, init_angles, init_ja_stride, init_wrist_xf,
                            init_xf_stride, mirror, t_scale, max_iters, n, joint_angles, ja_stride, wrist_xf, xf_stride},
                           weights, init_scale, scale_mode, scale, info};
  HIPCHK(h, ut::launch_fit_pose_scale(a, (hipStream_t)stream));
  return UT_OK;
}

int ut_pool_scale(ut_handle h, const float* scale, const float* info, int n_groups, int group_size, float* group,
                  float* pose_scale, void* stream) {
  if (n_groups == 0) return UT_OK;
  if (!scale || !info || !group || n_groups < 0 || group_size < 1) return fail(h, UT_E_INVALID, "ut_pool_scale: bad argument");
  ON_DEVICE_IF(h);
  HIPCHK(h, ut::launch_pool_scale(scale, info, n_groups, group_size, group, pose_scale, (hipStream_t)stream));
  return UT_OK;
}

struct ut_mesh {
  int device = 0;
  int n_vertices = 0, n_triangles = 0;
  void* verts = nullptr;
  uint32_t* csr_off = nullptr;
  uint32_t* csr_ent = nullptr;
  int32_t* tris = nullptr;
};
static_assert(UT_MESH_MAX_VERTICES == ut::MESH_MAX_VERTICES && UT_MESH_MAX_VERTICES <= 65536, "vertex cap");

int ut_mesh_create(const float* vertices, int n_vertices, const int32_t* triangles, int n_triangles,
                   const float* dense_bone_weights, int device, ut_mesh** out) {
  if (out) *out = nullptr;
  if (!out || !vertices || !dense_bone_weights || (!triangles && n_triangles != 0))
    return fail(nullptr, UT_E_INVALID, "ut_mesh_create: null argument");
  if (n_vertices <= 0) return fail(nullptr, UT_E_INVALID, "ut_mesh_create: the mesh has no vertices");
  if (n_triangles < 0) return fail(nullptr, UT_E_INVALID, "ut_mesh_create: negative triangle count");
  char msg[256];
  if (n_vertices > UT_MESH_MAX_VERTICES) {
    snprintf(msg, sizeof msg, "ut_mesh_create: %d vertices, more than UT_MESH_MAX_VERTICES (%d) that fit a workgroup's LDS",
             n_vertices, UT_MESH_MAX_VERTICES);
    return fail(nullptr, UT_E_UNSUPPORTED, msg);
  }
  if (n_triangles > (1 << 24)) return fail(nullptr, UT_E_UNSUPPORTED, "ut_mesh_create: more than 2^24 triangles");
  const size_t nv = (size_t)n_vertices, nt = (size_t)n_triangles;
  std::vector<float> packed(nv * 8, 0.f);
  for (size_t v = 0; v < nv; ++v) {
    float* p = &packed[v * 8];
    for (int k = 0; k < 3; ++k) {
      if (!std::isfinite(vertices[3 * v + k])) {
        snprintf(msg, sizeof msg, "ut_mesh_create: vertex %zu has a coordinate that is not finite", v);
        return fail(nullptr, UT_E_INVALID, msg);
      }
      p[k] = vertices[3 * v + k];
    }
    uint32_t bones = 0;
    int slots = 0;
    for (int f = 0; f < 17; ++f) {
      const float w = dense_bone_weights[17 * v + f];
      if (!std::isfinite(w)) {
        snprintf(msg, sizeof msg, "ut_mesh_create: weight [%zu][%d] is not finite", v, f);
        return fail(nullptr, UT_E_INVALID, msg);
      }
      if (w == 0.f) continue;
      if (slots == UT_MESH_MAX_INFLUENCES) {
        snprintf(msg, sizeof msg, "ut_mesh_create: vertex %zu has more than %d non-zero bone weights", v,
                 UT_MESH_MAX_INFLUENCES);
        return fail(nullptr, UT_E_UNSUPPORTED, msg);
      }
      bones |= (uint32_t)f << (8 * slots);
      p[4 + slots] = w;
      ++slots;
    }
    memcpy(&p[3], &bones, sizeof bones);
  }
  std::vector<uint32_t> off(nv + 1, 0), ent(nt * 3 + 1, 0);
  for (size_t t = 0; t < nt; ++t)
    for (int k = 0; k < 3; ++k) {
      const int32_t v = triangles[3 * t + k];
      if (v < 0 || v >= n_vertices) {
        snprintf(msg, sizeof msg, "ut_mesh_create: triangle %zu names vertex %d, outside [0, %d)", t, (int)v, n_vertices);
        return fail(nullptr, UT_E_INVALID, msg);
      }
      ++off[(size_t)v + 1];
    }
  for (size_t v = 0; v < nv; ++v) off[v + 1] += off[v];
  {
    std::vector<uint32_t> fill(off.begin(), off.end() - 1);
    for (size_t t = 0; t < nt; ++t)
      for (int k = 0; k < 3; ++k) {
        const uint32_t v = (uint32_t)triangles[3 * t + k];
        const uint32_t a = (uint32_t)triangles[3 * t + (k + 1) % 3], b = (uint32_t)triangles[3 * t + (k + 2) % 3];
        ent[fill[v]++] = a | (b << 16);
      }
  }
  std::vector<int32_t> tri4(nt * 4 + 4, 0);
  for (size_t t = 0; t < nt; ++t)
    for (int k = 0; k < 3; ++k) tri4[4 * t + k] = triangles[3 * t + k];
  DeviceScope scope(device);
  if (scope.err != hipSuccess) return fail(nullptr, UT_E_HIP, "hipSetDevice", scope.err);
  ut_mesh* m = new ut_mesh();
  m->device = device; m->n_vertices = n_vertices; m->n_triangles = n_triangles;
  hipError_t e = hipMalloc(&m->verts, packed.size() * sizeof(float));
  if (e == hipSuccess) e = hipMalloc((void**)&m->csr_off, off.size() * sizeof(uint32_t));
  if (e == hipSuccess) e = hipMalloc((void**)&m->csr_ent, ent.size() * sizeof(uint32_t));
  if (e == hipSuccess) e = hipMalloc((void**)&m->tris, tri4.size() * sizeof(int32_t));
  if (e == hipSuccess) e = hipMemcpy(m->tris, tri4.data(), tri4.size() * sizeof(int32_t), hipMemcpyHostToDevice);
  if (e == hipSuccess) e = hipMemcpy(m->verts, packed.data(), packed.size() * sizeof(float), hipMemcpyHostToDevice);
  if (e == hipSuccess) e = hipMemcpy(m->csr_off, off.data(), off.size() * sizeof(uint32_t), hipMemcpyHostToDevice);
  if (e == hipSuccess) e = hipMemcpy(m->csr_ent, ent.data(), ent.size() * sizeof(uint32_t), hipMemcpyHostToDevice);
  if (e != hipSuccess) {
    (void)hipFree(m->verts); (void)hipFree(m->csr_off); (void)hipFree(m->csr_ent); (void)hipFree(m->tris);
    delete m;
    return fail(nullptr, UT_E_HIP, "ut_mesh_create: upload", e);
  }
  *out = m;
  return UT_OK;
}

int ut_mesh_destroy(ut_mesh* m) {
  if (!m) return UT_OK;
  DeviceScope scope(m->device);
  (void)hipFree(m->verts); (void)hipFree(m->csr_off); (void)hipFree(m->csr_ent); (void)hipFree(m->tris);
  delete m;
  return UT_OK;
}

int ut_mesh_counts(const ut_mesh* m, int* n_vertices, int* n_triangles) {
  if (!m) return fail(nullptr, UT_E_INVALID, "ut_mesh_counts: null mesh");
  if (n_vertices) *n_vertices = m->n_vertices;
  if (n_triangles) *n_triangles = m->n_triangles;
  return UT_OK;
}

int ut_skin_mesh(ut_handle h, const ut_mesh* mesh, const float* hand_model, int n_models, const float* joint_angles,
                 int ja_stride, const float* wrist_xf, int xf_stride, const int64_t* mirror, float t_scale, int n,
                 float* out_vertices, float* out_normals, void* stream) {
  if (!mesh) return fail(h, UT_E_INVALID, "ut_skin_mesh: null mesh");
  if (h && h->device != mesh->device) return fail(h, UT_E_INVALID, "ut_skin_mesh: the mesh lives on another device than the handle");
  if (n == 0) return UT_OK;
  if (!hand_model || !joint_angles || !wrist_xf || !out_vertices || n < 0 || (n_models != 1 && n_models != n) ||
      ja_stride < 22 || xf_stride < 16)
    return fail(h, UT_E_INVALID, "ut_skin_mesh: bad argument");
  DeviceScope scope(mesh->device);
  if (scope.err != hipSuccess) return fail(h, UT_E_HIP, "hipSetDevice", scope.err);
  HIPCHK(h, ut::launch_skin_mesh(hand_model, n_models, joint_angles, ja_stride, wrist_xf, xf_stride, mirror, t_scale, n,
                                 mesh->verts, mesh->csr_off, mesh->csr_ent, mesh->n_vertices, out_vertices, out_normals,
                                 (hipStream_t)stream));
  return UT_OK;
}

namespace {
struct StatusTarget { int *dev = nullptr, *host = nullptr, mode = UT_CHECK_SYNC, device = 0; };
int status_target(ut_handle h, StatusTarget* t) {
  if (h) { t->dev = h->status; t->host = h->status_host; t->mode = h->check_mode; t->device = h->device; return UT_OK; }
  DevStatus st;
  int rc = stateless_status(&t->device, &st);
  if (rc) return rc;
  t->dev = st.dev; t->host = st.host;
  return UT_OK;
}
}

int ut_project_points(ut_handle h, const float* points, int point_stride, int n_points, const int32_t* cam_rows,
                      int max_views, const double* table, int n_rows, int table_kind, int n, int width, int height,
                      double* window, double* eye_z, uint8_t* flags, void* stream) {
  if (!points || !cam_rows || !table || !window || !eye_z || !flags)
    return fail(h, UT_E_INVALID, "ut_project_points: null argument");
  if (table_kind != UT_CAMERA_FISHEYE62 && table_kind != UT_CAMERA_PINHOLE)
    return fail(h, UT_E_INVALID, "ut_project_points: table_kind must be UT_CAMERA_FISHEYE62 or UT_CAMERA_PINHOLE");
  if (n < 0 || n_points <= 0 || max_views <= 0 || n_rows <= 0 || point_stride < 3 * n_points || width < 0 || height < 0)
    return fail(h, UT_E_INVALID, "ut_project_points: bad argument");
  if (n == 0) return UT_OK;
  StatusTarget st;
  int rc = status_target(h, &st);
  if (rc) return rc;
  DeviceScope scope(st.device);
  if (scope.err != hipSuccess) return fail(h, UT_E_HIP, "hipSetDevice", scope.err);
  hipStream_t s = (hipStream_t)stream;
  ut::ProjectArgs g{};
  g.points = points; g.point_stride = point_stride; g.n_points = n_points; g.cam_rows = cam_rows; g.max_views = max_views;
  g.table = table; g.n_rows = n_rows; g.kind = table_kind == UT_CAMERA_FISHEYE62 ? ut::PROJECT_FISHEYE62 : ut::PROJECT_PINHOLE;
  g.n = n; g.width = width; g.height = height; g.window = window; g.eye_z = eye_z; g.flags = flags; g.status = st.dev;
  HIPCHK(h, ut::launch_project_points(g, s));
  return st.mode == UT_CHECK_SYNC ? check_status(h, st.dev, st.host, s, "ut_project_points") : UT_OK;
}

static_assert(UT_TRI_MAX_VIEWS == ut::TRI_MAX_VIEWS && UT_TRI_CONVERGED == ut::TRI_CONVERGED && UT_TRI_AT_MAX_ITERS == ut::TRI_AT_MAX_ITERS &&
              UT_TRI_REFUSED == ut::TRI_REFUSED && UT_TRI_DEGENERATE == ut::TRI_DEGENERATE, "triangulation constants");

namespace {
int triangulate_points(ut_handle h, const char* who, const double* window, const float* weights, const int32_t* cam_rows,
                       int max_views, const double* table, int n_rows, int table_kind, int n_points, int n, int max_iters,
                       double* points, float* points_f32, int point_stride, float* info, float* residual, float* sqrt_info,
                       void* stream) {
  if (!window || !cam_rows || !table) return fail_as(h, who, "null argument");
  if (!points && !points_f32) return fail_as(h, who, "one of points and points_f32 must be given");
  if (table_kind != UT_CAMERA_FISHEYE62 && table_kind != UT_CAMERA_PINHOLE)
    return fail_as(h, who, "table_kind must be UT_CAMERA_FISHEYE62 or UT_CAMERA_PINHOLE");
  if (max_views < 1 || max_views > UT_TRI_MAX_VIEWS) return fail_as(h, who, "max_views must be in 1..UT_TRI_MAX_VIEWS (8)");
  if (max_iters < 1 || max_iters > 64) return fail_as(h, who, "max_iters must be in 1..64");
  if (n < 0 || n_points < 1 || n_rows < 1 || (points_f32 && point_stride < 3 * n_points)) return fail_as(h, who, "bad argument");
  if (n == 0) return UT_OK;
  if (h) {
    hipPointerAttribute_t attr;
    if (hipPointerGetAttributes(&attr, window) == hipSuccess && attr.type == hipMemoryTypeDevice && attr.device != h->device)
      return fail_as(h, who, "the windows live on another device than the handle");
  }
  StatusTarget st;
  int rc = status_target(h, &st);
  if (rc) return rc;
  DeviceScope scope(st.device);
  if (scope.err != hipSuccess) return fail(h, UT_E_HIP, "hipSetDevice", scope.err);
  hipStream_t s = (hipStream_t)stream;
  ut::TriArgs g{};
  g.window = window; g.weights = weights; g.cam_rows = cam_rows; g.max_views = max_views; g.table = table; g.n_rows = n_rows;
  g.kind = table_kind == UT_CAMERA_FISHEYE62 ? ut::PROJECT_FISHEYE62 : ut::PROJECT_PINHOLE;
  g.n_points = n_points; g.n = n; g.max_iters = max_iters; g.points = points; g.points_f32 = points_f32;
  g.point_stride = point_stride; g.info = info; g.residual = residual; g.status = st.dev; g.sqrt_info = sqrt_info;
  HIPCHK(h, ut::launch_triangulate(g, s));
  return st.mode == UT_CHECK_SYNC ? check_status(h, st.dev, st.host, s, who) : UT_OK;
}
}

int ut_triangulate_points(ut_handle h, const double* window, const float* weights, const int32_t* cam_rows, int max_views,
                          const double* table, int n_rows, int table_kind, int n_points, int n, int max_iters,
                          double* points, float* points_f32, int point_stride, float* info, float* residual, void* stream) {
  return triangulate_points(h, "ut_triangulate_points", window, weights, cam_rows, max_views, table, n_rows, table_kind, n_points,
                            n, max_iters, points, points_f32, point_stride, info, residual, nullptr, stream);
}

int ut_triangulate_points_info(ut_handle h, const double* window, const float* weights, const int32_t* cam_rows, int max_views,
                               const double* table, int n_rows, int table_kind, int n_points, int n, int max_iters,
                               double* points, float* points_f32, int point_stride, float* info, float* residual,
                               float* sqrt_info, void* stream) {
  if (!sqrt_info) return fail(h, UT_E_INVALID, "ut_triangulate_points_info: null argument");
  return triangulate_points(h, "ut_triangulate_points_info", window, weights, cam_rows, max_views, table, n_rows, table_kind,
                            n_points, n, max_iters, points, points_f32, point_stride, info, residual, sqrt_info, stream);
}

int ut_fit_pose_views(ut_handle h, const float* hand_model, int n_models, const double* window, const float* weights,
                      const int32_t* cam_rows, int max_views, const double* table, int n_rows, int table_kind, const float* limits,
                      const float* init_angles, int init_ja_stride, const float* init_wrist_xf, int init_xf_stride,
                      const int64_t* mirror, float t_scale, int max_iters, int n, float* joint_angles, int ja_stride,
                      float* wrist_xf, int xf_stride, float* info, float* residual, void* stream) {
  const char* who = "ut_fit_pose_views";
  if (!window || !cam_rows || !table) return fail_as(h, who, "null argument");
  if (table_kind != UT_CAMERA_FISHEYE62 && table_kind != UT_CAMERA_PINHOLE)
    return fail_as(h, who, "table_kind must be UT_CAMERA_FISHEYE62 or UT_CAMERA_PINHOLE");
  if (max_views < 1 || max_views > UT_TRI_MAX_VIEWS) return fail_as(h, who, "max_views must be in 1..UT_TRI_MAX_VIEWS (8)");
  if (n_rows < 1) return fail_as(h, who, "bad argument");
  const int rc = fit_pose_args(h, who, hand_model, n_models, nullptr, 0, init_angles, init_ja_stride, init_wrist_xf,
                               init_xf_stride, t_scale, max_iters, n, joint_angles, ja_stride, wrist_xf, xf_stride, false);
  if (rc) return rc;
  if (n == 0) return UT_OK;
  if (h) {
    hipPointerAttribute_t attr;
    if (hipPointerGetAttributes(&attr, window) == hipSuccess && attr.type == hipMemoryTypeDevice && attr.device != h->device)
      return fail_as(h, who, "the windows live on another device than the handle");
  }
  StatusTarget st;
  const int rs = status_target(h, &st);
  if (rs) return rs;
  DeviceScope scope(st.device);
  if (scope.err != hipSuccess) return fail(h, UT_E_HIP, "hipSetDevice", scope.err);
  hipStream_t s = (hipStream_t)stream;
  const ut::FitViewsArgs a{{hand_model, n_models, nullptr, 0, limits, init_angles, init_ja_stride, init_wrist_xf, init_xf_stride,
                            mirror, t_scale, max_iters, n, joint_angles, ja_stride, wrist_xf, xf_stride},
                           window, weights, cam_rows, max_views, table, n_rows,
                           table_kind == UT_CAMERA_FISHEYE62 ? ut::PROJECT_FISHEYE62 : ut::PROJECT_PINHOLE, info, residual, st.dev};
  HIPCHK(h, ut::launch_fit_pose_views(a, s));
  return st.mode == UT_CHECK_SYNC ? check_status(h, st.dev, st.host, s, who) : UT_OK;
}

static_assert(UT_RENDER_MAX_VERTICES == ut::RENDER_MAX_VERTICES && UT_RENDER_MAX_VERTICES <= UT_MESH_MAX_VERTICES, "vertex cap");

int ut_render_mesh(ut_handle h, const ut_mesh* mesh, const float* vertices, const double* crop_params, int n_crops,
                   const int64_t* sample_range, int n, int crop_size, float* depth, int32_t* tri, uint8_t* shade,
                   void* stream) {
  if (!mesh) return fail(h, UT_E_INVALID, "ut_render_mesh: null mesh");
  if (h && h->device != mesh->device) return fail(h, UT_E_INVALID, "ut_render_mesh: the mesh lives on another device than the handle");
  if (mesh->n_triangles <= 0) return fail(h, UT_E_INVALID, "ut_render_mesh: the mesh has no triangles");
  if (crop_size != ut::RENDER_CROP) return fail(h, UT_E_UNSUPPORTED, "ut_render_mesh: crop_size must be 96");
  if (mesh->n_vertices > UT_RENDER_MAX_VERTICES) {
    char msg[200];
    snprintf(msg, sizeof msg, "ut_render_mesh: %d vertices, more than UT_RENDER_MAX_VERTICES (%d) that fit a workgroup's LDS next "
             "to the depth plane", mesh->n_vertices, UT_RENDER_MAX_VERTICES);
    return fail(h, UT_E_UNSUPPORTED, msg);
  }
  if (n < 0 || n_crops < 0) return fail(h, UT_E_INVALID, "ut_render_mesh: bad argument");
  if (n == 0) return UT_OK;
  if (!vertices || !crop_params || !sample_range) return fail(h, UT_E_INVALID, "ut_render_mesh: null argument");
  if (((uintptr_t)depth | (uintptr_t)tri | (uintptr_t)shade) & 15)
    return fail(h, UT_E_INVALID, "ut_render_mesh: depth, tri and shade must be 16-byte aligned");
  DeviceScope scope(mesh->device);
  if (scope.err != hipSuccess) return fail(h, UT_E_HIP, "hipSetDevice", scope.err);
  StatusTarget st;
  int rc = status_target(h, &st);
  if (rc) return rc;
  hipStream_t s = (hipStream_t)stream;
  ut::RenderArgs g{};
  g.vertices = vertices; g.nv = mesh->n_vertices; g.tris = (const int4*)mesh->tris; g.nt = mesh->n_triangles;
  g.crop_params = crop_params; g.sample_range = sample_range; g.n = n; g.n_crops = n_crops;
  g.depth = depth; g.tri = tri; g.shade = shade; g.status = st.dev;
  HIPCHK(h, ut::launch_render_check(g, s));
  if (st.mode == UT_CHECK_SYNC && (rc = check_status(h, st.dev, st.host, s, "ut_render_mesh"))) return rc;
  HIPCHK(h, ut::launch_render_mesh(g, s));
  return UT_OK;
}

int ut_gen_crop_cameras(ut_handle h, const double* cam_params, const double* camera_angles, const float* hand_model,
                        const float* joint_limits, int n_models, const float* joint_angles, const float* wrist_xf,
                        const int32_t* frame_idx, const int64_t* hand_idx, int n, int n_cams, int max_views, int min_vis,
                        int src_w, int src_h, int crop_size, double focal_multiplier, double* crop_params,
                        float* intrinsics, float* extrinsics, int32_t* cam_index, int32_t* n_views, int32_t* status,
                        float* landmarks, void* stream) {
  if (n == 0) return UT_OK;
  if (!cam_params || !camera_angles || !hand_model || !joint_limits || !joint_angles || !wrist_xf || !frame_idx ||
      !hand_idx || !crop_params || !intrinsics || !extrinsics || !cam_index || !n_views || !status || n < 0 ||
      (n_models != 1 && n_models != n) || n_cams <= 0 || max_views <= 0 || src_w <= 0 || src_h <= 0 || crop_size <= 1)
    return fail(h, UT_E_INVALID, "ut_gen_crop_cameras: bad argument");
  ON_DEVICE_IF(h);
  ut::CropGenArgs g{};
  g.cam_params = cam_params; g.camera_angles = camera_angles; g.hand_model = hand_model; g.joint_limits = joint_limits;
  g.joint_angles = joint_angles; g.wrist_xf = wrist_xf; g.frame_idx = frame_idx; g.hand_idx = hand_idx;
  g.n = n; g.n_models = n_models; g.n_cams = n_cams; g.max_views = max_views; g.min_vis = min_vis;
  g.src_w = src_w; g.src_h = src_h; g.crop_size = crop_size; g.focal_multiplier = focal_multiplier;
  g.crop_params = crop_params; g.intrinsics = intrinsics; g.extrinsics = extrinsics; g.cam_index = cam_index;
  g.n_views = n_views; g.status = status; g.landmarks = landmarks;
  HIPCHK(h, ut::launch_cropgen(g, (hipStream_t)stream));
  return UT_OK;
}

int ut_gen_crop_cameras_from_window_points(ut_handle h, const double* cam_params, int n_cam_rows, const double* keypoints,
                                           const int32_t* src_row, const int64_t* hand_idx, int n, int max_views,
                                           int crop_size, double focal_multiplier, double* crop_params, float* intrinsics,
                                           float* extrinsics, int32_t* cam_index, int32_t* n_views, int32_t* status,
                                           void* stream) {
  if (n == 0) return UT_OK;
  if (!cam_params || !keypoints || !src_row || !hand_idx || !crop_params || !intrinsics || !extrinsics || !cam_index ||
      !n_views || !status || n < 0 || n_cam_rows <= 0 || max_views < 1 || max_views > 3 || crop_size <= 1)
    return fail(h, UT_E_INVALID, "ut_gen_crop_cameras_from_window_points: bad argument");
  ON_DEVICE_IF(h);
  std::vector<int32_t> rows((size_t)n * max_views);
  std::vector<int64_t> hands((size_t)n);
  HIPCHK(h, hipMemcpyAsync(rows.data(), src_row, rows.size() * sizeof(int32_t), hipMemcpyDefault, (hipStream_t)stream));
  HIPCHK(h, hipMemcpyAsync(hands.data(), hand_idx, hands.size() * sizeof(int64_t), hipMemcpyDefault, (hipStream_t)stream));
  HIPCHK(h, hipStreamSynchronize((hipStream_t)stream));
  for (int32_t r : rows)
    if (r < -1 || r >= n_cam_rows)
      return fail(h, UT_E_INVALID, "ut_gen_crop_cameras_from_window_points: src_row outside [-1, n_cam_rows)");
  for (int64_t x : hands)
    if (x != 0 && x != 1) return fail(h, UT_E_INVALID, "ut_gen_crop_cameras_from_window_points: hand_idx not 0 or 1");
  ut::CropGenWindowArgs g{};
  g.cam_params = cam_params; g.keypoints = keypoints; g.src_row = src_row; g.hand_idx = hand_idx;
  g.n = n; g.max_views = max_views; g.crop_size = crop_size; g.focal_multiplier = focal_multiplier;
  g.crop_params = crop_params; g.intrinsics = intrinsics; g.extrinsics = extrinsics; g.cam_index = cam_index;
  g.n_views = n_views; g.status = status;
  HIPCHK(h, ut::launch_cropgen_window(g, (hipStream_t)stream));
  return UT_OK;
}

int ut_gen_crop_matrices(ut_handle h, const float* orig_extrinsics, const float* orig_intrinsics, const float* crop_points,
                         const int64_t* hand_idx, int n_frames, int n_views, int n_pts, int crop_size,
                         double focal_multiplier, float* extrinsics_xf, float* new_intrinsics, float* resample_xf,
                         int32_t* status, void* stream) {
  if (n_frames == 0 || n_views == 0) return UT_OK;
  if (!orig_extrinsics || !orig_intrinsics || !crop_points || !hand_idx || !extrinsics_xf || !new_intrinsics ||
      !resample_xf || !status || n_frames < 0 || n_views < 0 || n_pts <= 0 || crop_size <= 1)
    return fail(h, UT_E_INVALID, "ut_gen_crop_matrices: bad argument");
  ON_DEVICE_IF(h);
  ut::CropMatArgs g{};
  g.orig_extrinsics = orig_extrinsics; g.orig_intrinsics = orig_intrinsics; g.crop_points = crop_points;
  g.hand_idx = hand_idx; g.n_frames = n_frames; g.n_views = n_views; g.n_pts = n_pts; g.crop_size = crop_size;
  g.focal_multiplier = focal_multiplier; g.extrinsics_xf = extrinsics_xf; g.new_intrinsics = new_intrinsics;
  g.resample_xf = resample_xf; g.status = status;
  HIPCHK(h, ut::launch_cropmat(g, (hipStream_t)stream));
  return UT_OK;
}

int ut_resample_homography(ut_handle h, const void* src, int src_is_f32, int n, int src_h, int src_w,
                           const float* resample_xf, int out_h, int out_w, float* out, void* stream) {
  if (n == 0) return UT_OK;
  if (!src || !resample_xf || !out || n < 0 || src_h < 2 || src_w < 2 || out_h <= 0 || out_w <= 0)
    return fail(h, UT_E_INVALID, "ut_resample_homography: bad argument");
  ON_DEVICE_IF(h);
  HIPCHK(h, ut::launch_resample_homography(src, src_is_f32, n, src_h, src_w, resample_xf, out_h, out_w, out,
                                           (hipStream_t)stream));
  return UT_OK;
}

int ut_keypoint_metrics(ut_handle h, const float* gt, const float* tracked, const uint8_t* valid, int n_hands, int n_frames,
                        double* err, double* acc, double* gt_acc, uint8_t* valid_acc, void* stream) {
  if (n_hands == 0 || n_frames == 0) return UT_OK;
  if (!gt || !tracked || !valid || !err || n_hands < 0 || n_frames < 0 ||
      (n_frames >= 3 && (!acc || !gt_acc || !valid_acc)))
    return fail(h, UT_E_INVALID, "ut_keypoint_metrics: bad argument");
  ON_DEVICE_IF(h);
  HIPCHK(h, ut::launch_keypoint_metrics(gt, tracked, valid, n_hands, n_frames, err, acc, gt_acc, valid_acc,
                                        (hipStream_t)stream));
  return UT_OK;
}

int ut_set_backbone_lanes(ut_handle h, int lanes) {
  if (!h || (lanes != 1 && lanes != 2)) return fail(h, UT_E_INVALID, "ut_set_backbone_lanes: 1 or 2");
  h->lanes = lanes;
  return UT_OK;
}

int ut_set_conv_arithmetic(ut_handle h, int mode) {
  if (!h || (mode != UT_CONV_FP32 && mode != UT_CONV_SPLIT_F16 && mode != UT_CONV_SPLIT_F16_ALWAYS)) return fail(h, UT_E_INVALID, "ut_set_conv_arithmetic: bad argument");
  h->conv_arith = mode;
  if (mode != UT_CONV_FP32 && h->scale_mode != UT_SPLIT_SCALE_DYNAMIC && !h->calibrated) {
    ON_DEVICE_OF(h);
    return calibrate_builtin(h);
  }
  return UT_OK;
}

int ut_set_block_fusion(ut_handle h, int on) {
  if (!h) return UT_E_INVALID;
  h->block_fusion = on != 0;
  return UT_OK;
}

int ut_set_resident_weights(ut_handle h, int on) {
  if (!h) return UT_E_INVALID;
  if (on < 0 || on > 6) return fail(h, UT_E_INVALID, "ut_set_resident_weights: bad argument");
  h->resident_weights = on;
  return UT_OK;
}

int ut_set_latency_mode(ut_handle h, int on) {
  if (!h) return UT_E_INVALID;
  ON_DEVICE_OF(h);
  if (on && !h->splitk_ws) {
    const size_t n = 1u << 20;
    int rc;
    if ((rc = dev_alloc(h, &h->splitk_ws, n)) || (rc = dev_alloc(h, &h->zero_bias, 256))) return rc;
    HIPCHK(h, hipMemset(h->zero_bias, 0, 256 * sizeof(float)));
    h->splitk_floats = n;
  }
  h->latency_mode = on != 0;
  return UT_OK;
}

int ut_set_index_checks(ut_handle h, int mode) {
  if (!h || (mode != UT_CHECK_SYNC && mode != UT_CHECK_DEFERRED)) return fail(h, UT_E_INVALID, "ut_set_index_checks: bad argument");
  h->check_mode = mode;
  return UT_OK;
}

int ut_poll_status(ut_handle h, void* stream) {
  if (!h) return UT_E_INVALID;
  ON_DEVICE_OF(h);
  return check_status(h, h->status, h->status_host, (hipStream_t)stream, "reported late (deferred checks)");
}

int ut_status_snapshot(ut_handle h, int32_t* dst, void* stream) {
  if (!h || !dst) return fail(h, UT_E_INVALID, "ut_status_snapshot: null argument");
  ON_DEVICE_OF(h);
  HIPCHK(h, hipMemcpyAsync(dst, h->status, 2 * sizeof(int), hipMemcpyDeviceToDevice, (hipStream_t)stream));
  return UT_OK;
}

int ut_profile_begin(ut_handle h, void* stream) {
  if (!h) return UT_E_INVALID;
  (void)stream;
  ON_DEVICE_OF(h);
  prof_clear(h);
  h->profiling = true;
  return UT_OK;
}

int ut_profile_end(ut_handle h, void* stream, double* conv_ms_total, int64_t* conv_launches, double* conv_flops_total) {
  if (!h) return UT_E_INVALID;
  ON_DEVICE_OF(h);
  double ms[2], fl[2];
  int64_t n[2];
  int rc = prof_reduce(h, (hipStream_t)stream, ms, n, fl);
  if (rc) return rc;
  if (conv_ms_total) *conv_ms_total = ms[0] + ms[1];
  if (conv_launches) *conv_launches = n[0] + n[1];
  if (conv_flops_total) *conv_flops_total = fl[0] + fl[1];
  return UT_OK;
}

int ut_profile_end_by_kind(ut_handle h, void* stream, double* ms2, int64_t* launches2, double* flops2) {
  if (!h || !ms2 || !launches2 || !flops2) return UT_E_INVALID;
  ON_DEVICE_OF(h);
  return prof_reduce(h, (hipStream_t)stream, ms2, launches2, flops2);
}

}
```

### absolutetrack_amd/csrc/ut_kernels.h

```cpp
#pragma once
#include <hip/hip_runtime.h>
#include <stdint.h>

#include "ut_split_pack.h"

namespace ut {

struct ConvLaunch {
  const float* in;
  const float* w;
  const void* w_split;
  float split_unscale;
  int* status;
  const unsigned* in_max;
  const unsigned* in_obs;
  int split_adaptive;
  unsigned* adapt_count;
  unsigned* out_max;
  const float* bias;
  const float* res;
  float* out;
  int n_img, H, W, cin, Ho, Wo;
  int cout_store;
  int cout_pad;
  int k_total;
  int k_cin;
  int cslice;
  int k_pad;
  int ksize, stride, pad;
  int relu;
  int out_nchw;
  int device;
  int num_cu;
  unsigned* tile_counter;
  int no_resident;
  int splits;
};

hipError_t launch_conv_igemm(const ConvLaunch& c, hipStream_t s);
hipError_t launch_splitk_finish(const float* slabs, int n_splits, int m, int cout_store, const float* bias,
                                const float* res, float* out, int relu, hipStream_t s);
struct PwLayer {
  const float* w;
  const float* bias;
  int k_pad, cout_store, cout_pad;
  int relu;
};
struct PwLaunch {
  const float* in;
  float* out;
  PwLayer layer[3];
  int n_layers;
  int n_img, H, W, cin, Ho, Wo, stride;
  int cout_store;
  int out_nchw;
  int num_cu;
};
bool conv_pw_applicable(const PwLaunch& c);
hipError_t launch_conv_pw(const PwLaunch& c, hipStream_t s);
bool conv_split_applicable(const ConvLaunch& c);
hipError_t launch_conv_split(const ConvLaunch& c, hipStream_t s);
struct Stride2Launch {
  const float* in;
  float* out1;
  float* out2;
  const void* w1_split;
  const void* wd_split;
  float unscale1, unscale_d;
  const float* bias1;
  const float* bias_d;
  const unsigned* in_max;
  const unsigned* in_obs;
  int split_adaptive;
  unsigned* adapt_count;
  unsigned* out1_max;
  int* status;
  int n_img, H, W;
  int device, num_cu;
};
bool conv_c32s2_applicable(const Stride2Launch& c);
hipError_t launch_conv_c32s2(const Stride2Launch& c, hipStream_t s);
enum W4Form : int { W4_NONE = 0, W4_TILES128, W4_MAP24, W4_STRIDE2 };
W4Form conv_w4_form(const ConvLaunch& c);
hipError_t launch_conv_w4(const ConvLaunch& c, hipStream_t s);
bool conv_c64k_applicable(const ConvLaunch& c);
hipError_t launch_conv_c64k(const ConvLaunch& c, hipStream_t s);
struct BlockLaunch {
  const float* in;
  float* out;
  const void* w1_split;
  const void* w2_split;
  float unscale_w1, unscale_w2;
  const float* bias1;
  const float* bias2;
  float wsum1;
  float bmax1;
  const unsigned* in_max;
  const unsigned* in_obs;
  int split_adaptive;
  unsigned* adapt_count;
  unsigned* out_max;
  int* status;
  unsigned* tile_counter;
  int n_img, H, W, device, num_cu;
};
bool conv_block32_applicable(const BlockLaunch& b);
hipError_t launch_conv_block32(const BlockLaunch& b, hipStream_t s);

hipError_t launch_zero_words(void* p, size_t n_words, hipStream_t s);
hipError_t launch_merge_max(unsigned* dst, const unsigned* src, hipStream_t s);
hipError_t launch_raise_words(unsigned* words, int n, int add_exp, hipStream_t s);
hipError_t launch_calibration_crops(float* crops, int n, hipStream_t s);
bool conv_patch_applicable(const ConvLaunch& c);
hipError_t launch_conv_patch(const ConvLaunch& c, hipStream_t s);

enum ConvKernel : int { CONV_IGEMM = 0, CONV_PATCH, CONV_SPLIT, CONV_W4, CONV_C64K };
constexpr const char* kConvKernelName[5] = {"conv_igemm", "conv_patch", "conv_split", "conv_w4", "conv_c64k"};

enum : int {
  NO_C64K = 1,
  NO_W4 = 2,
  NO_W4_MAP24 = 4,
  NO_W4_STRIDE2 = 8,
};
constexpr int kResidentKinds[7] = {
    NO_C64K | NO_W4 | NO_W4_MAP24 | NO_W4_STRIDE2,
    0,
    NO_W4 | NO_W4_MAP24 | NO_W4_STRIDE2,
    NO_C64K | NO_W4_STRIDE2,
    NO_W4_MAP24 | NO_W4_STRIDE2,
    NO_C64K | NO_W4_MAP24 | NO_W4_STRIDE2,
    NO_W4_STRIDE2,
};

inline bool conv_prefers_patch(const ConvLaunch& c) {
  const long m = (long)c.n_img * c.Ho * c.Wo;
  const bool few_tiles = ((m + 63) / 64) * ((c.cout_store + 63) / 64) <= (long)c.num_cu;
  return conv_patch_applicable(c) && !(c.splits == 1 && few_tiles);
}

inline ConvKernel choose_conv(const ConvLaunch& c) {
  if (c.splits > 1) return CONV_IGEMM;
  if (c.w_split && conv_split_applicable(c)) {
    const int off = c.no_resident;
    const W4Form form = conv_w4_form(c);
    const int form_bit = form == W4_MAP24 ? NO_W4_MAP24 : form == W4_STRIDE2 ? NO_W4_STRIDE2 : 0;
    if (form != W4_NONE && !(off & (NO_W4 | form_bit))) return CONV_W4;
    if (conv_c64k_applicable(c) && !(off & NO_C64K)) return CONV_C64K;
    return CONV_SPLIT;
  }
  return conv_prefers_patch(c) ? CONV_PATCH : CONV_IGEMM;
}

inline hipError_t launch_conv_on(ConvKernel k, const ConvLaunch& c, hipStream_t s) {
  switch (k) {
    case CONV_PATCH: return launch_conv_patch(c, s);
    case CONV_SPLIT: return launch_conv_split(c, s);
    case CONV_W4: return launch_conv_w4(c, s);
    case CONV_C64K: return launch_conv_c64k(c, s);
    default: return launch_conv_igemm(c, s);
  }
}
inline hipError_t launch_conv(const ConvLaunch& c, hipStream_t s, ConvKernel* ran = nullptr) {
  const ConvKernel k = choose_conv(c);
  if (ran) *ran = k;
  return launch_conv_on(k, c, s);
}

hipError_t launch_stem(const float* crops, const float* w , const float* bias ,
                       float* out, int n, unsigned* out_max, hipStream_t s);
hipError_t launch_stem_u8(const uint8_t* crops, const float* w, const float* bias, float* out, int n, unsigned* out_max,
                          hipStream_t s);

struct HeadBuffers {
  float* cat144;
  float* f108;
  float* f72a;
  float* f72b;
  float* fused;
  float* t92a;
  float* t92b;
  float* regin;
  float* rega;
  float* regb;
  float* skel;
  float* xf;
};

enum : int {
  UT_BAD_SAMPLE_RANGE = 1,
  UT_BAD_MEMORY_IDX = 2,
  UT_DUP_MEMORY_IDX = 4,
  UT_BAD_HAND_IDX = 8,
  UT_SINGLE_VIEW = 16,
  UT_BAD_SRC_INDEX = 32,
  UT_SPLIT_RANGE = 64,
};
constexpr int UT_STATUS_ERRORS = UT_BAD_SAMPLE_RANGE | UT_BAD_MEMORY_IDX | UT_DUP_MEMORY_IDX | UT_BAD_HAND_IDX | UT_BAD_SRC_INDEX | UT_SPLIT_RANGE;

#if defined(__HIPCC__)
__device__ __forceinline__ unsigned abs_bits(float v) { return __float_as_uint(v) & 0x7FFFFFFFu; }

__device__ __forceinline__ void publish_abs_max(unsigned* word, unsigned lane_bits) {
#pragma unroll
  for (int o = 32; o; o >>= 1) {
    const unsigned other = (unsigned)__shfl_xor((int)lane_bits, o);
    lane_bits = other > lane_bits ? other : lane_bits;
  }
  if ((threadIdx.x & 63) == 0 && lane_bits > __hip_atomic_load(word, __ATOMIC_RELAXED, __HIP_MEMORY_SCOPE_AGENT))
    atomicMax(word, lane_bits);
}

__device__ __forceinline__ int split_pow2_for(int e, bool none, float& scale, float& unscale) {
  int k = none ? 0 : 141 - e;
  k = k > 100 ? 100 : k < -100 ? -100 : k;
  scale = __uint_as_float((unsigned)(127 + k) << 23);
  unscale = __uint_as_float((unsigned)(127 - k) << 23);
  return k;
}

__device__ __forceinline__ unsigned split_act_scale(const unsigned* in_max, const unsigned* in_obs, bool adaptive, float& scale,
                                                    float& unscale, bool& ok, bool& adapted) {
  unsigned bits = (unsigned)__builtin_amdgcn_readfirstlane((int)*in_max);
  const unsigned obs = in_obs ? (unsigned)__builtin_amdgcn_readfirstlane((int)*in_obs) : 0u;
  const int eo = (int)(obs >> 23);
  int e = (int)(bits >> 23);
  int k = split_pow2_for(e, bits == 0u || e == 255, scale, unscale);
  adapted = adaptive && in_obs && obs != 0u && eo != 255 && (eo + k > 142 || eo + 11 < e);
  if (adapted) {
    bits = obs;
    e = eo;
    k = split_pow2_for(e, false, scale, unscale);
  }
  ok = e != 255;
  if (in_obs && !adapted && (eo == 255 || eo + k > 142)) ok = false;
  return bits;
}

__device__ __forceinline__ void split_scale_report(bool ok, bool adapted, int* status, unsigned* adapt_count) {
  if (threadIdx.x == 0 && blockIdx.x == 0) {
    if (!ok && status) atomicOr(status, UT_SPLIT_RANGE);
    if (adapted && adapt_count) atomicAdd(adapt_count, 1u);
  }
}
#endif

struct HeadArgs {
  const float* feat;
  const float* intrinsics;
  const float* extrinsics;
  const int64_t* sample_range;
  const int64_t* memory_idx;
  const uint8_t* use_memory;
  const int64_t* hand_idx;
  int n_samples;
  int n_crops;
  int n_slots;
  float* mem;
  float* prev_ext;
  int* status;
  int call_error_mask;
  int* slot_seen;
};

hipError_t launch_validate_desc(const HeadArgs& a, hipStream_t s);

hipError_t launch_ftl_in(const HeadArgs& a, const HeadBuffers& b, bool staged, hipStream_t s);
hipError_t launch_ftl_out_temporal_in(const HeadArgs& a, const HeadBuffers& b, hipStream_t s);
hipError_t launch_temporal_out(const HeadArgs& a, const float* t_out , const float* skel,
                               int n_skel, float* regin, int reg_c, int reg_stride, unsigned* out_max, hipStream_t s);
hipError_t launch_skeleton(const float* skel_in , const float* w ,
                           const float* bias , const float* bn_scale ,
                           const float* bn_shift , float* out , int n_skel,
                           hipStream_t s);
hipError_t launch_pool_decode(const HeadArgs& a, const float* reg_feat , int reg_c, int reg_stride,
                              const float* w , const float* bias , int d,
                              float* out_pose, float* out_raw, float* raw_ws , hipStream_t s);

hipError_t launch_fk(const float* hand_model, int n_models, const float* ja, int ja_stride,
                     const float* xf, int xf_stride, const int64_t* mirror, float t_scale, int n,
                     float* out, hipStream_t s);

struct FitPoseArgs {
  const float* hand_model; int n_models;
  const float* targets; int target_stride;
  const float* limits;
  const float* init_ja; int init_ja_stride;
  const float* init_xf; int init_xf_stride;
  const int64_t* mirror;
  float t_scale;
  int max_iters, n;
  float* ja; int ja_stride;
  float* xf; int xf_stride;
};
enum : int { FIT_CONVERGED = 1, FIT_AT_MAX_ITERS = 2, FIT_REFUSED = 4 };

struct FitArgs {
  FitPoseArgs pose;
  const float* weights;
  float* info;
};
hipError_t launch_fit_pose(const FitArgs& a, hipStream_t s);

struct FitInfoArgs {
  FitPoseArgs pose;
  const float* sqrt_info;
  float* info;
};
hipError_t launch_fit_pose_info(const FitInfoArgs& a, hipStream_t s);

struct FitViewsArgs {
  FitPoseArgs pose;
  const double* window;
  const float* weights;
  const int32_t* cam_rows;
  int max_views;
  const double* table;
  int n_rows, kind;
  float* info;
  float* residual;
  int* status;
};
hipError_t launch_fit_pose_views(const FitViewsArgs& a, hipStream_t s);

constexpr int FITS_MODE_FREE = 0, FITS_MODE_FIXED = 1;
constexpr float FITS_SCALE_MIN = 0.25f, FITS_SCALE_MAX = 4.0f, FITS_SCALE_INFO_LAMBDA = 1e-6f;
enum : int { FITS_CONVERGED = FIT_CONVERGED, FITS_AT_MAX_ITERS = FIT_AT_MAX_ITERS, FITS_REFUSED = FIT_REFUSED, FITS_AT_BOUND = 8 };
struct FitScaleArgs {
  FitPoseArgs pose;
  const float* weights;
  const float* init_scale;
  int scale_mode;
  float* scale;
  float* info;
};
hipError_t launch_fit_pose_scale(const FitScaleArgs& a, hipStream_t s);
hipError_t launch_pool_scale(const float* scale, const float* info, int n_groups, int group_size, float* group,
                             float* pose_scale, hipStream_t s);

constexpr int MESH_MAX_VERTICES = 5056;
hipError_t launch_skin_mesh(const float* hand_model, int n_models, const float* ja, int ja_stride, const float* xf,
                            int xf_stride, const int64_t* mirror, float t_scale, int n, const void* verts,
                            const uint32_t* csr_off, const uint32_t* csr_ent, int nv, float* out_v, float* out_n,
                            hipStream_t s);

enum : int { PROJECT_FISHEYE62 = 0, PROJECT_PINHOLE = 1 };
struct ProjectArgs {
  const float* points;
  int point_stride, n_points;
  const int32_t* cam_rows;
  int max_views;
  const double* table;
  int n_rows, kind, n;
  int width, height;
  double* window;
  double* eye_z;
  uint8_t* flags;
  int* status;
};
hipError_t launch_project_points(const ProjectArgs& g, hipStream_t s);

constexpr int TRI_MAX_VIEWS = 8;
enum : int { TRI_CONVERGED = 1, TRI_AT_MAX_ITERS = 2, TRI_REFUSED = 4, TRI_DEGENERATE = 8 };
struct TriArgs {
  const double* window;
  const float* weights;
  const int32_t* cam_rows;
  int max_views;
  const double* table;
  int n_rows, kind, n_points, n, max_iters;
  double* points;
  float* points_f32;
  int point_stride;
  float* info;
  float* residual;
  int* status;
  float* sqrt_info;
};
hipError_t launch_triangulate(const TriArgs& a, hipStream_t s);

constexpr int RENDER_CROP = 96;
constexpr int RENDER_MAX_VERTICES = 2368;
struct RenderArgs {
  const float* vertices;
  int nv;
  const int4* tris;
  int nt;
  const double* crop_params;
  const int64_t* sample_range;
  int n, n_crops;
  float* depth;
  int32_t* tri;
  uint8_t* shade;
  int* status;
};
hipError_t launch_render_check(const RenderArgs& g, hipStream_t s);
hipError_t launch_render_mesh(const RenderArgs& g, hipStream_t s);

struct CropGenArgs {
  const double* cam_params;
  const double* camera_angles;
  const float* hand_model;
  const float* joint_limits;
  const float* joint_angles;
  const float* wrist_xf;
  const int32_t* frame_idx;
  const int64_t* hand_idx;
  int n, n_models, n_cams, max_views, min_vis, src_w, src_h, crop_size;
  double focal_multiplier;
  double* crop_params;
  float* intrinsics;
  float* extrinsics;
  int32_t* cam_index;
  int32_t* n_views;
  int32_t* status;
  float* landmarks;
};
hipError_t launch_cropgen(const CropGenArgs& g, hipStream_t s);

struct CropGenWindowArgs {
  const double* cam_params;
  const double* keypoints;
  const int32_t* src_row;
  const int64_t* hand_idx;
  int n, max_views, crop_size;
  double focal_multiplier;
  double* crop_params;
  float* intrinsics;
  float* extrinsics;
  int32_t* cam_index;
  int32_t* n_views;
  int32_t* status;
};
hipError_t launch_cropgen_window(const CropGenWindowArgs& g, hipStream_t s);

struct CropMatArgs {
  const float* orig_extrinsics;
  const float* orig_intrinsics;
  const float* crop_points;
  const int64_t* hand_idx;
  int n_frames, n_views, n_pts, crop_size;
  double focal_multiplier;
  float* extrinsics_xf;
  float* new_intrinsics;
  float* resample_xf;
  int32_t* status;
};
hipError_t launch_cropmat(const CropMatArgs& g, hipStream_t s);
hipError_t launch_resample_homography(const void* src, int src_is_f32, int n, int src_h, int src_w,
                                      const float* resample_xf, int out_h, int out_w, float* out, hipStream_t s);

hipError_t launch_keypoint_metrics(const float* gt, const float* tracked, const uint8_t* valid, int n_hands, int n_frames,
                                   double* err, double* acc, double* gt_acc, uint8_t* valid_acc, hipStream_t s);

hipError_t launch_mem_export(const float* mem , float* out , int slots, hipStream_t s);

hipError_t launch_warp(const uint8_t* src, int n_src, int src_h, int src_w, const double* cam,
                       const double* crop, const int32_t* src_index, int n_crops, int mode, float* out,
                       uint8_t* out_u8, int* status, hipStream_t s);

hipError_t launch_warp_map(const double* cam, const double* crop, const int32_t* src_index, int n_src, int n_crops,
                           float* out, hipStream_t s);

}
```

Measured before the change: 168,300 hand-frames/s.

## Chain consecutive stride-1 W4 convolutions into one persistent multi-layer launch

Adds a chained form of the persistent W4 conv kernel that walks several consecutive same-shape layers in one launch. Blocks take tiles layer by layer, swap buffer descriptors, bias and scales per layer, and prefetch the next layer's inputs and weights while the current epilogue runs. A per-layer scale table is precomputed in LDS. The host queues eligible convs into a chain and flushes it at boundaries. The aim is to remove per-layer launch gaps and the tail idle time between layers, at the cost of cross-layer dependency handling, extra waits, and added complexity in the kernel and the host.

```diff
diff --git a/absolutetrack_amd/csrc/conv_w4.hip b/absolutetrack_amd/csrc/conv_w4.hip
--- a/absolutetrack_amd/csrc/conv_w4.hip
+++ b/absolutetrack_amd/csrc/conv_w4.hip
@@ -1,3 +1,5 @@
+#include <type_traits>
+
 #include "ut_kernels.h"
 #include "ut_conv_dev.h"
 
@@ -14,11 +16,13 @@
 static_assert(9 % W4_NSET == 0, "the register sets of the weight fragments line up across slices");
 constexpr int w4_cap(int pixels, int wi, int hi) { return ((pixels / (wi * hi)) * (hi + 1) * (wi + 1) + 2 * (wi + 2) + 15) / 16 * 16; }
 
-template <int WI, int HI, int SCH, int WPX, bool S2 = false>
-__global__ __launch_bounds__(256, 1) void conv_w4_kernel(ConvLaunch p, int tiles_n, int n_tiles) {
+template <int WI, int HI, int SCH, int WPX, bool S2 = false, bool CHAIN = false>
+__global__ __launch_bounds__(256, 1) void conv_w4_kernel(typename std::conditional<CHAIN, W4ChainLaunch, ConvLaunch>::type p, int tiles_n, int n_tiles) {
   extern __shared__ __attribute__((aligned(16))) char smem[];
   constexpr int MI = W4_MI, PW = WI + 1, PH = HI + 1, HW = WI * HI;
   static_assert(!S2 || (SCH == 32 && WPX == 1), "phase planes: two 16-channel planes per buffer, four 32-channel blocks per tile");
+  static_assert(!(S2 && CHAIN), "chains: the stride-1 forms");
+  constexpr int LDAUX = CHAIN ? 16 : 0;
   constexpr int BM = W4_WPIX * WPX;
   constexpr int NCB = 4 / WPX, BN = 32 * NCB;
   constexpr int NG = SCH / 4, NHG = NG / 2;
@@ -30,7 +34,8 @@
   constexpr int GSTRIDE = CAP * 16;
   constexpr int STAGE = NG * GSTRIDE;
   constexpr int SLOT = NBUF * STAGE;
-  constexpr int EPI = SLOT + 16;
+  constexpr int KTAB = SLOT + 16;
+  constexpr int EPI = SLOT + (CHAIN ? 64 : 16);
   static_assert(BM % HW == 0, "a tile is a whole number of maps: every tile has the same padded layout");
   static_assert(BM * NG == W4_NLOAD * 256 && KS % W4_NSET == 0 && (SCH == 32 || SCH == 16) && (WPX == 1 || WPX == 2), "shape");
   static_assert((NG - 2) * GSTRIDE + (2 * PW + 2) * 16 < 65536, "fragment reads: everything but the lane's base fits the immediate offset");
@@ -43,16 +48,16 @@
   const int fr = lane & 31, fh = lane >> 5;
 
   const int M = p.n_img * HW;
-  const int n_slices = (!S2 && p.k_cin > 0 ? p.k_cin : p.cin) / (S2 ? 16 : SCH);
+  int n_slices = (!S2 && p.k_cin > 0 ? p.k_cin : p.cin) / (S2 ? 16 : SCH);
   const int n_chunks = p.k_pad / 32;
 
-  const __amdgpu_buffer_rsrc_t a_rsrc = __builtin_amdgcn_make_buffer_rsrc(
+  __amdgpu_buffer_rsrc_t a_rsrc = __builtin_amdgcn_make_buffer_rsrc(
       const_cast<float*>(p.in), 0, (int)((size_t)M * (S2 ? 4 : 1) * p.cin * sizeof(float)), 0x00020000);
-  const __amdgpu_buffer_rsrc_t w_rsrc = __builtin_amdgcn_make_buffer_rsrc(
+  __amdgpu_buffer_rsrc_t w_rsrc = __builtin_amdgcn_make_buffer_rsrc(
       const_cast<void*>(p.w_split), 0, (int)((size_t)(p.cout_pad / 32) * n_chunks * 4096), 0x00020000);
-  const __amdgpu_buffer_rsrc_t r_rsrc = __builtin_amdgcn_make_buffer_rsrc(
+  __amdgpu_buffer_rsrc_t r_rsrc = __builtin_amdgcn_make_buffer_rsrc(
       const_cast<float*>(p.res ? p.res : p.bias), 0, p.res ? (int)((size_t)M * p.cout_store * sizeof(float)) : 0, 0x00020000);
-  const __amdgpu_buffer_rsrc_t o_rsrc =
+  __amdgpu_buffer_rsrc_t o_rsrc =
       __builtin_amdgcn_make_buffer_rsrc(p.out, 0, (int)((size_t)M * p.cout_store * sizeof(float)), 0x00020000);
   const __amdgpu_buffer_rsrc_t q_rsrc = __builtin_amdgcn_make_buffer_rsrc(p.tile_counter, 0, 4, 0x00020000);
 
@@ -62,8 +67,15 @@
     split_act_scale(p.in_max, p.in_obs, p.split_adaptive, x_scale, x_unscale, ok, adapted);
     split_scale_report(ok, adapted, p.status, p.adapt_count);
   }
-  const float tot_unscale = p.split_unscale * x_unscale;
-  const float floor_v = p.relu ? 0.f : -__builtin_huge_valf();
+  float tot_unscale = p.split_unscale * x_unscale;
+  float floor_v = p.relu ? 0.f : -__builtin_huge_valf();
+  const float* bias_c = p.bias;
+  unsigned* out_max_c = p.out_max;
+  int guard_k = 0;
+  bool guarded = false;
+  float xs_n = x_scale;
+  __amdgpu_buffer_rsrc_t a_rsrc_n = a_rsrc, w_rsrc_n = w_rsrc;
+  int n_slices_n = n_slices;
   const unsigned row_b = (unsigned)p.cout_store * 4u;
 
   const int grid = gridDim.x;
@@ -83,6 +95,7 @@
   }
   const unsigned h_step = (unsigned)(RP * p.cin) * 4u;
 #define W4_H_BASE(TILE) ((unsigned)((((TILE) / tiles_n) * BM + tid / NG) * p.cin + 4 * (tid % NG)) * 4u)
+#define W4_H_BASE_U(UNIT) ((unsigned)(((UNIT) * BM + tid / NG) * p.cin + 4 * (tid % NG)) * 4u)
   unsigned h_in[S2 ? W4_NLOAD : 1], po_a = 0, po_b = 0, pb1[S2 ? MI : 1];
   if constexpr (S2) {
 #pragma unroll
@@ -106,11 +119,12 @@
 
 #define W4_READ_X(I, PC, S, TAP, BASE)                                                               \
   xp[I][PC] = *reinterpret_cast<const u32x4*>(smem + (BASE)[I] + (unsigned)(((PC) * NHG + (SCH == 32 ? 2 * (S) : 0)) * GSTRIDE + (((TAP) / 3) * PW + (TAP) % 3) * 16));
-#define W4_LOAD_W(SET, PL, CH, S, WROW)                                                              \
+#define W4_LOAD_W_OF(RS, SET, PL, CH, S, WROW)                                                       \
   {                                                                                                  \
     const unsigned so_ = (WROW) + (unsigned)((wco * n_chunks + (CH)) * 4096 + ((S) * 2 + (PL)) * 1024); \
-    wf[SET][PL] = __builtin_bit_cast(u32x4, __builtin_amdgcn_raw_buffer_load_b128(w_rsrc, w_lane, so_, 0)); \
-  }
+    wf[SET][PL] = __builtin_bit_cast(u32x4, __builtin_amdgcn_raw_buffer_load_b128(RS, w_lane, so_, 0)); \
+  }
+#define W4_LOAD_W(SET, PL, CH, S, WROW) W4_LOAD_W_OF(w_rsrc, SET, PL, CH, S, WROW)
 #define W4S_PLANE(Q) ((0x190 >> (Q)) & 1)
 #define W4S_TAPP(Q) ((int)((0x414344310ull >> (4 * (Q))) & 15))
 #define W4S_TAPO(Q) ((int)((0x715348620ull >> (4 * (Q))) & 15))
@@ -141,18 +155,34 @@
   int cur_buf = 0;
   unsigned out_bits = 0;
   const unsigned slot_addr = (unsigned)(unsigned long)(lds_char*)smem + (unsigned)SLOT;
+  const int tn_sh = tiles_n == 2 ? 1 : 0, tn_mask = tiles_n - 1;
+  int u_c = slot, s_c = 0, u_o = -1, s_o = 0, nx_u = -1, nx_s = 0, adv_u = -1, adv_s = 0, k_c = 0, k_n = 0;
+  bool dep = false;
+  int steps = 0;
+  if constexpr (CHAIN) {
+    steps = p.n_layers << tn_sh;
+    u_o = grid + slot < n_tiles ? grid + slot : -1;
+    if (tid < p.n_layers) {
+      const unsigned bits = *p.lay[tid].in_max;
+      const int e = (int)(bits >> 23);
+      float sc_, un_;
+      *reinterpret_cast<int*>(smem + KTAB + 4 * tid) = split_pow2_for(e, bits == 0u || e == 255, sc_, un_);
+      if (tid > 0 && e == 255 && blockIdx.x == 0 && p.status) atomicOr(p.status, UT_SPLIT_RANGE);
+    }
+  }
 
   for (int k = tid; k < NBUF * STAGE / 16; k += 256) *reinterpret_cast<u32x4*>(smem + k * 16) = u32x4{0, 0, 0, 0};
   __syncthreads();
-  unsigned h_base = S2 ? 0u : W4_H_BASE(tile);
-  unsigned w_row = (unsigned)((tile % tiles_n) * NCB) * (unsigned)n_chunks * 4096u;
+  unsigned h_base = S2 ? 0u : CHAIN ? W4_H_BASE_U(slot) : W4_H_BASE(tile);
+  unsigned w_row = CHAIN ? 0u : (unsigned)((tile % tiles_n) * NCB) * (unsigned)n_chunks * 4096u;
   unsigned w_row_next = w_row;
+  if constexpr (CHAIN) k_c = k_n = slot_read(slot_addr + (unsigned)(KTAB - SLOT));
   if constexpr (!S2) {
 #pragma unroll
     for (int a = 0; a < AHEAD; ++a)
 #pragma unroll
       for (int j = 0; j < W4_NLOAD; ++j) {
-        const float4 v = __builtin_bit_cast(float4, __builtin_amdgcn_raw_buffer_load_b128(a_rsrc, h_base + (unsigned)j * h_step, (unsigned)(a * SCH * 4), 0));
+        const float4 v = __builtin_bit_cast(float4, __builtin_amdgcn_raw_buffer_load_b128(a_rsrc, h_base + (unsigned)j * h_step, (unsigned)(a * SCH * 4), LDAUX));
         if (a == AHEAD - 1 && KS == 9 && j >= W4_NLOAD - 4) stg[j % W4_NSTG] = v;
         else W4_SPLIT_STORE(v, (unsigned)(a * STAGE) + h_wa[j])
       }
@@ -189,26 +219,26 @@
           if ((N) >= 19 && (N) <= 26 && q1 < KS) { W4_READ_X(((N) + 8) % 9, 0, W4_HALF(sl, q1), W4_TAP(q1), rb) } \
           if ((N) >= 19 && (N) <= 26 && q1 == KS) { W4_READ_X(((N) + 8) % 9, 0, 0, 0, nb) }          \
           if (((N) == 10 || (N) == 11) && qd < KS) { W4_LOAD_W(qd % W4_NSET, (N) & 1, W4_CHUNK(sl, qd), W4_HALF(sl, qd), w_row) } \
-          if (((N) == 10 || (N) == 11) && qd >= KS) { W4_LOAD_W(qd % W4_NSET, (N) & 1, W4_CHUNK(sl_after, qd - KS), W4_HALF(sl_after, qd - KS), row_after) } \
-          if ((N) == 12 && q >= 4 && q < 4 + W4_NLOAD) { const float4 v_ = stg[(q + W4_NSTG - 4) % W4_NSTG]; split_pair_scaled(v_.x, v_.y, x_scale, cv0, cv1); } \
+          if (((N) == 10 || (N) == 11) && qd >= KS) { W4_LOAD_W_OF(wr_after, qd % W4_NSET, (N) & 1, W4_CHUNK(sl_after, qd - KS), W4_HALF(sl_after, qd - KS), row_after) } \
+          if ((N) == 12 && q >= 4 && q < 4 + W4_NLOAD) { const float4 v_ = stg[(q + W4_NSTG - 4) % W4_NSTG]; split_pair_scaled(v_.x, v_.y, xs_f, cv0, cv1); } \
           if ((N) == 13 && q >= 4 && q < 4 + W4_NLOAD) {                                             \
             const float4 v_ = stg[(q + W4_NSTG - 4) % W4_NSTG];                                      \
             unsigned a1_, b1_;                                                                       \
-            split_pair_scaled(v_.z, v_.w, x_scale, a1_, b1_);                                        \
+            split_pair_scaled(v_.z, v_.w, xs_f, a1_, b1_);                                           \
             *reinterpret_cast<u32x2*>(smem + wbuf + h_wa[(q + 5) % 9]) = u32x2{cv0, a1_};            \
             *reinterpret_cast<u32x2*>(smem + wbuf + h_wa[(q + 5) % 9] + NHG * GSTRIDE) = u32x2{cv1, b1_}; \
           }                                                                                          \
-          if (KS == 9 && (N) == 12 && q < 4) { const float4 v_ = stg[q % W4_NSTG]; split_pair_scaled(v_.x, v_.y, x_scale, cv0, cv1); } \
+          if (KS == 9 && (N) == 12 && q < 4) { const float4 v_ = stg[q % W4_NSTG]; split_pair_scaled(v_.x, v_.y, xs_p, cv0, cv1); } \
           if (KS == 9 && (N) == 13 && q < 4) {       \
             const float4 v_ = stg[q % W4_NSTG];                                                      \
             unsigned a1_, b1_;                                                                       \
-            split_pair_scaled(v_.z, v_.w, x_scale, a1_, b1_);                                        \
+            split_pair_scaled(v_.z, v_.w, xs_p, a1_, b1_);                                           \
             *reinterpret_cast<u32x2*>(smem + pbuf + h_wa[q + 5]) = u32x2{cv0, a1_};                  \
             *reinterpret_cast<u32x2*>(smem + pbuf + h_wa[q + 5] + NHG * GSTRIDE) = u32x2{cv1, b1_};  \
           }                                                                                          \
           if ((N) == 14 && q < W4_NLOAD)                                                             \
-            stg[q % W4_NSTG] = __builtin_bit_cast(float4, __builtin_amdgcn_raw_buffer_load_b128(a_rsrc, h_base + (unsigned)q * h_step, f_soff, 0)); \
-          if ((N) == 16 && q == KS / 2 && sl == 0 && tid == 0) *reinterpret_cast<int*>(smem + SLOT) = grid + ticket; \
+            stg[q % W4_NSTG] = __builtin_bit_cast(float4, __builtin_amdgcn_raw_buffer_load_b128(f_rsrc, h_base + (unsigned)q * h_step, f_soff, LDAUX)); \
+          if ((N) == 16 && q == KS / 2 && sl == 0 && tid == 0) *reinterpret_cast<int*>(smem + SLOT) = (CHAIN ? 2 * grid : grid) + ticket; \
           W4_PIN();                                                                                  \
           W4_MFMA(ws, N);                                                                            \
           W4_PIN();                                                                                  \
@@ -222,10 +252,14 @@
         if (q == KS - 1) {                                                                           \
                                        \
           W4_READ_X(MI - 1, 0, W4_HALF(sl, KS - 1), 8, rb)                                           \
+                                                                            \
+          if (CHAIN && sl == 0) asm volatile("s_waitcnt vmcnt(0)" ::: "memory");                     \
           asm volatile("s_waitcnt lgkmcnt(0)" ::: "memory");                                         \
           __builtin_amdgcn_s_barrier();                                                              \
           asm volatile("" ::: "memory");                                                             \
-          if (sl == 0) {                                                                             \
+          if constexpr (CHAIN) {                                                                     \
+            if (sl == 0) { W4_CHAIN_NEXT() }                                                         \
+          } else if (sl == 0) {                                                                      \
             next_tile = slot_read(slot_addr);                                                        \
             w_row_next = (unsigned)((next_tile % tiles_n) * NCB) * (unsigned)n_chunks * 4096u;       \
           }                                                                                          \
@@ -297,15 +331,56 @@
         W4S_SLOT_BODY(18) W4S_SLOT_BODY(19) W4S_SLOT_BODY(20) W4S_SLOT_BODY(21) W4S_SLOT_BODY(22) W4S_SLOT_BODY(23) W4S_SLOT_BODY(24) W4S_SLOT_BODY(25) W4S_SLOT_BODY(26) \
       }
 
+#define W4_CHAIN_NEXT()                                                                              \
+  {                                                                                                  \
+    const int l_c = s_c >> tn_sh;                                                                    \
+    const bool fresh = s_c + 1 == steps, two = u_o >= 0;                                             \
+    adv_s = fresh ? 0 : s_c + 1;                                                                     \
+    nx_s = two ? s_o : adv_s;                                                                        \
+    const int l_n = nx_s >> tn_sh, l_g = l_c + 1 < p.n_layers ? l_c + 1 : l_c;                       \
+    int tk_, kn_, kg_;                                                                               \
+    asm volatile("ds_read_b32 %0, %3\n\tds_read_b32 %1, %4\n\tds_read_b32 %2, %5\n\ts_waitcnt lgkmcnt(0)" \
+                 : "=&v"(tk_), "=&v"(kn_), "=&v"(kg_)                                                \
+                 : "v"(slot_addr), "v"(slot_addr + (unsigned)(KTAB - SLOT + 4 * l_n)), "v"(slot_addr + (unsigned)(KTAB - SLOT + 4 * l_g)) : "memory"); \
+    const int tk = __builtin_amdgcn_readfirstlane(tk_);                                              \
+    adv_u = fresh ? ((unsigned)tk < (unsigned)n_tiles ? tk : -1) : u_c;                              \
+    nx_u = two ? u_o : adv_u;                                                                        \
+    dep = !two && !fresh && (adv_s & tn_mask) == 0;                                                  \
+    guarded = l_c + 1 < p.n_layers;                                                                  \
+    guard_k = __builtin_amdgcn_readfirstlane(kg_);                                                   \
+    const unsigned o_bytes = (unsigned)M * (unsigned)p.cout_store * 4u;                              \
+    {                                                                                                \
+      const W4Layer& lc = p.lay[l_c];                                                                \
+      r_rsrc = __builtin_amdgcn_make_buffer_rsrc(const_cast<float*>(lc.res ? lc.res : lc.bias), 0, lc.res ? (int)o_bytes : 0, 0x00020000); \
+      o_rsrc = __builtin_amdgcn_make_buffer_rsrc(lc.out, 0, (int)o_bytes, 0x00020000);               \
+      bias_c = lc.bias;                                                                              \
+      out_max_c = lc.out_max;                                                                        \
+      tot_unscale = lc.split_unscale * __uint_as_float((unsigned)(127 - k_c) << 23);                 \
+      floor_v = lc.relu ? 0.f : -__builtin_huge_valf();                                              \
+      bb4 = *reinterpret_cast<const float4*>(bias_c + (s_c & tn_mask) * BN + wco * 32 + 4 * (lane & 7)); \
+    }                                                                                                \
+    if (nx_u >= 0) {                                                                                 \
+      const W4Layer& ln = p.lay[l_n];                                                                \
+      a_rsrc_n = __builtin_amdgcn_make_buffer_rsrc(const_cast<float*>(ln.in), 0, (int)((unsigned)M * (unsigned)p.cin * 4u), 0x00020000); \
+      w_rsrc_n = __builtin_amdgcn_make_buffer_rsrc(const_cast<void*>(ln.w_split), 0, (int)((size_t)(p.cout_pad / 32) * n_chunks * 4096), 0x00020000); \
+      k_n = __builtin_amdgcn_readfirstlane(kn_);                                                     \
+      xs_n = __uint_as_float((unsigned)(127 + k_n) << 23);                                           \
+      n_slices_n = (ln.k_cin > 0 ? ln.k_cin : p.cin) / SCH;                                          \
+      w_row_next = (unsigned)((nx_s & tn_mask) * NCB) * (unsigned)n_chunks * 4096u;                  \
+    }                                                                                                \
+  }
+
   for (;;) {
     int ticket = 0;
-    if (tid == 0) ticket = __builtin_amdgcn_raw_ptr_buffer_atomic_add_i32(1, q_rsrc, 0, 0, 0);
+    if (tid == 0 && (!CHAIN || s_c + 1 == steps)) ticket = __builtin_amdgcn_raw_ptr_buffer_atomic_add_i32(1, q_rsrc, 0, 0, 0);
+    if constexpr (CHAIN) out_bits = 0;
 #pragma unroll
     for (int i = 0; i < MI; ++i)
 #pragma unroll
       for (int e = 0; e < 16; ++e) acc[i][e] = 0.f;
 
-    const float4 bb4 = *reinterpret_cast<const float4*>(p.bias + (tile % tiles_n) * BN + wco * 32 + 4 * (lane & 7));
+    float4 bb4 = float4{0.f, 0.f, 0.f, 0.f};
+    if constexpr (!CHAIN) bb4 = *reinterpret_cast<const float4*>(p.bias + (tile % tiles_n) * BN + wco * 32 + 4 * (lane & 7));
     if constexpr (S2) {
       for (int sl = 0; sl < n_slices; ++sl) {
         const bool last_slice = sl == n_slices - 1;
@@ -324,10 +399,15 @@
       unsigned wbuf = (unsigned)__builtin_amdgcn_readfirstlane((NBUF == 2 ? b1 : b2) * STAGE), pbuf = nbuf;
       asm volatile("" : "+s"(rbuf), "+s"(nbuf), "+s"(wbuf), "+s"(pbuf));
       const int f_sl = sl + AHEAD < n_slices ? sl + AHEAD : sl + AHEAD - n_slices;
-      if (sl + AHEAD == n_slices) h_base = W4_H_BASE(next_tile);
+      if constexpr (CHAIN) {
+        if (sl + AHEAD == n_slices) h_base = nx_u >= 0 && !dep ? W4_H_BASE_U(nx_u) : W4_HOOB;
+      } else if (sl + AHEAD == n_slices) h_base = W4_H_BASE(next_tile);
       const unsigned f_soff = (unsigned)f_sl * (SCH * 4);
       const int sl_after = last_slice ? 0 : sl + 1;
       const unsigned row_after = last_slice ? w_row_next : w_row;
+      const bool f_next = CHAIN && sl + AHEAD >= n_slices, p_next = CHAIN && sl > 0 && sl - 1 + AHEAD >= n_slices;
+      const float xs_f = f_next ? xs_n : x_scale, xs_p = p_next ? xs_n : x_scale;
+      const __amdgpu_buffer_rsrc_t f_rsrc = f_next ? a_rsrc_n : a_rsrc, wr_after = CHAIN && last_slice ? w_rsrc_n : w_rsrc;
       unsigned rb[MI], nb[MI];
 #pragma unroll
       for (int i = 0; i < MI; ++i) { rb[i] = pb[i] + rbuf; nb[i] = pb[i] + nbuf; }
@@ -335,10 +415,10 @@
       cur_buf = b1;
     }
     {
-      const int tm = tile / tiles_n, tn = tile - tm * tiles_n;
+      const int tm = CHAIN ? u_c : tile / tiles_n, tn = CHAIN ? s_c & tn_mask : tile - tm * tiles_n;
       const bool ragged = tm * BM + BM > M;
       const int ch = tn * BN + wco * 32 + fr;
-      const float bb = p.bias[ch];
+      const float bb = bias_c[ch];
       const unsigned base = ch < p.cout_store ? (unsigned)((tm * BM + wm * W4_WPIX + 4 * fh) * p.cout_store + ch) * 4u : W4_HOOB;
       const unsigned keep_n = base != W4_HOOB ? 0x7FFFFFFFu : 0u;
       if (!ragged) {
@@ -353,7 +433,7 @@
           for (int i = 0; i < 5; ++i)
 #pragma unroll
             for (int t = 0; t < 4; ++t)
-              rr[i][t] = __builtin_bit_cast(float4, __builtin_amdgcn_raw_buffer_load_b128(r_rsrc, base4, (unsigned)(32 * i + 8 * t) * row_bs, 0));
+              rr[i][t] = __builtin_bit_cast(float4, __builtin_amdgcn_raw_buffer_load_b128(r_rsrc, base4, (unsigned)(32 * i + 8 * t) * row_bs, LDAUX));
         }
         char* const ex = smem + EPI + wave * 4096;
 #define W4_EX_WRITE(H)                                                                               \
@@ -366,7 +446,7 @@
           if (!S2 && (h & 1) == 0 && i + 5 < MI) {
 #pragma unroll
             for (int t = 0; t < 4; ++t)
-              rr[(i + 5) % 6][t] = __builtin_bit_cast(float4, __builtin_amdgcn_raw_buffer_load_b128(r_rsrc, base4, (unsigned)(32 * (i + 5) + 8 * t) * row_bs, 0));
+              rr[(i + 5) % 6][t] = __builtin_bit_cast(float4, __builtin_amdgcn_raw_buffer_load_b128(r_rsrc, base4, (unsigned)(32 * (i + 5) + 8 * t) * row_bs, LDAUX));
           }
           if (h + 1 < 2 * MI) { W4_EX_WRITE(h + 1) }
 #pragma unroll
@@ -393,7 +473,7 @@
           unsigned off = base + (unsigned)(i * 32) * row_b;
 #pragma unroll
           for (int r = 0; r < 16; ++r) {
-            r1[r] = __uint_as_float(__builtin_amdgcn_raw_buffer_load_b32(r_rsrc, off, 0, 0));
+            r1[r] = __uint_as_float(__builtin_amdgcn_raw_buffer_load_b32(r_rsrc, off, 0, LDAUX));
             off += ((r & 3) == 3 ? 5u : 1u) * row_b;
           }
           off = base + (unsigned)(i * 32) * row_b;
@@ -408,12 +488,64 @@
         }
       }
     }
-    if ((unsigned)next_tile >= (unsigned)n_tiles) break;
-    tile = next_tile;
-    w_row = w_row_next;
-  }
-  if (p.out_max) publish_abs_max(p.out_max, out_bits);
+    if constexpr (CHAIN) {
+      {
+        unsigned wb = out_bits;
+#pragma unroll
+        for (int o = 32; o; o >>= 1) {
+          const unsigned other = (unsigned)__shfl_xor((int)wb, o);
+          wb = other > wb ? other : wb;
+        }
+        if (lane == 0) {
+          if (out_max_c && wb > __hip_atomic_load(out_max_c, __ATOMIC_RELAXED, __HIP_MEMORY_SCOPE_AGENT)) atomicMax(out_max_c, wb);
+          const int eo = (int)(wb >> 23);
+          if (guarded && (eo == 255 || eo + guard_k > 142) && p.status) atomicOr(p.status, UT_SPLIT_RANGE);
+        }
+      }
+      if (nx_u < 0) break;
+      const bool two = u_o >= 0;
+      u_c = nx_u; s_c = nx_s;
+      if (two) { u_o = adv_u; s_o = adv_s; }
+      a_rsrc = a_rsrc_n; w_rsrc = w_rsrc_n; x_scale = xs_n; k_c = k_n; n_slices = n_slices_n;
+      w_row = w_row_next;
+      if (dep) {
+        asm volatile("s_waitcnt vmcnt(0)" ::: "memory");
+        __syncthreads();
+        h_base = W4_H_BASE_U(u_c);
+        int bo = cur_buf;
+#pragma unroll
+        for (int a = 0; a < AHEAD; ++a) {
+          const unsigned dst = (unsigned)__builtin_amdgcn_readfirstlane(bo * STAGE);
+#pragma unroll
+          for (int j = 0; j < W4_NLOAD; ++j) {
+            const float4 v = __builtin_bit_cast(float4, __builtin_amdgcn_raw_buffer_load_b128(a_rsrc, h_base + (unsigned)j * h_step, (unsigned)(a * SCH * 4), LDAUX));
+            if (a == AHEAD - 1 && KS == 9 && j >= W4_NLOAD - 4) stg[j % W4_NSTG] = v;
+            else W4_SPLIT_STORE(v, dst + h_wa[j])
+          }
+          bo = bo + 1 == NBUF ? 0 : bo + 1;
+        }
+        __syncthreads();
+        const unsigned rb0 = (unsigned)__builtin_amdgcn_readfirstlane(cur_buf * STAGE);
+        unsigned rb[MI];
+#pragma unroll
+        for (int i = 0; i < MI; ++i) rb[i] = pb[i] + rb0;
+#pragma unroll
+        for (int i = 0; i < MI; ++i) {
+          W4_READ_X(i, 1, 0, 0, rb)
+          if (i < MI - 1) { W4_READ_X(i, 0, 0, 0, rb) }
+        }
+      }
+    } else {
+      if ((unsigned)next_tile >= (unsigned)n_tiles) break;
+      tile = next_tile;
+      w_row = w_row_next;
+    }
+  }
+  if constexpr (!CHAIN) { if (p.out_max) publish_abs_max(p.out_max, out_bits); }
 #undef W4_H_BASE
+#undef W4_H_BASE_U
+#undef W4_LOAD_W_OF
+#undef W4_CHAIN_NEXT
 #undef W4_READ_X
 #undef W4_LOAD_W
 #undef W4_TAP
@@ -449,6 +581,15 @@
   return launch_with_lds<&conv_w4_kernel<WI, HI, SCH, WPX, S2>>(c.device, lds, persistent_grid(c.num_cu, n_tiles), 256, s, c, tiles_n, n_tiles);
 }
 
+template <int WI, int HI, int SCH, int WPX>
+hipError_t launch_w4_chain_cfg(const W4ChainLaunch& c, hipStream_t s) {
+  constexpr int BM = W4_WPIX * WPX, BN = 128 / WPX;
+  const long M = (long)c.n_img * c.Ho * c.Wo;
+  const int units = (int)((M + BM - 1) / BM), tiles_n = c.cout_store / BN;
+  constexpr int lds = (SCH == 32 ? 2 : 3) * (SCH / 4) * w4_cap(BM, WI, HI) * 16 + 64 + 4 * 4096;
+  return launch_with_lds<&conv_w4_kernel<WI, HI, SCH, WPX, false, true>>(c.device, lds, persistent_grid(c.num_cu, units), 256, s, c, tiles_n, units);
+}
+
 }
 
 W4Form conv_w4_form(const ConvLaunch& c) {
@@ -474,4 +615,36 @@
   return c.W == 12 ? launch_w4_cfg<12, 12, 32, 1>(c, s) : launch_w4_cfg<6, 6, 32, 1>(c, s);
 }
 
-}
+
+bool conv_w4_chainable(const ConvLaunch& a, const ConvLaunch& b) {
+  const W4Form fa = conv_w4_form(a), fb = conv_w4_form(b);
+  if (fa != fb || (fa != W4_TILES128 && fa != W4_MAP24)) return false;
+  if (a.cout_store > 256 || a.cin != a.cout_store) return false;
+  return b.in == a.out && b.in_obs == a.out_max && a.out_max && b.in_max && a.in_max && !a.split_adaptive && !b.split_adaptive &&
+         a.n_img == b.n_img && a.H == b.H && a.W == b.W && a.cin == b.cin && a.cout_store == b.cout_store && a.cout_pad == b.cout_pad &&
+         a.k_pad == b.k_pad && a.status == b.status && a.device == b.device && a.num_cu == b.num_cu;
+}
+
+bool conv_w4_chain_fills(const ConvLaunch& c) {
+  const long units = ((long)c.n_img * c.Ho * c.Wo + W4_WPIX - 1) / W4_WPIX;
+  return c.cout_store <= 128 || units >= (long)c.num_cu;
+}
+
+hipError_t launch_conv_w4_chain(const ConvLaunch* layers, int n_layers, hipStream_t s) {
+  if (n_layers < 1 || n_layers > W4_MAX_CHAIN) return hipErrorInvalidValue;
+  for (int l = 1; l < n_layers; ++l)
+    if (!conv_w4_chainable(layers[l - 1], layers[l])) return hipErrorInvalidValue;
+  const W4Form form = conv_w4_form(layers[0]);
+  if ((form != W4_TILES128 && form != W4_MAP24) || !layers[0].in_max || !layers[0].out_max) return hipErrorInvalidValue;
+  W4ChainLaunch c{};
+  static_cast<ConvLaunch&>(c) = layers[0];
+  c.n_layers = n_layers;
+  for (int l = 0; l < n_layers; ++l) {
+    const ConvLaunch& a = layers[l];
+    c.lay[l] = W4Layer{a.in, a.res, a.out, a.w_split, a.bias, a.in_max, a.out_max, a.split_unscale, a.k_cin, a.relu};
+  }
+  if (form == W4_MAP24) return launch_w4_chain_cfg<24, 24, 16, 2>(c, s);
+  return c.W == 12 ? launch_w4_chain_cfg<12, 12, 32, 1>(c, s) : launch_w4_chain_cfg<6, 6, 32, 1>(c, s);
+}
+
+}
diff --git a/absolutetrack_amd/csrc/ut_api.hip b/absolutetrack_amd/csrc/ut_api.hip
--- a/absolutetrack_amd/csrc/ut_api.hip
+++ b/absolutetrack_amd/csrc/ut_api.hip
@@ -49,6 +49,7 @@
 };
 
 struct ProfEvent { hipEvent_t a, b; double flops;   int kind = 0;
+  int convs = 1;
 };
 
 }
@@ -89,6 +90,9 @@
   unsigned word_gen = 0;
   bool block_fusion = true;
   int resident_weights = 1;
+  std::vector<ut::ConvLaunch> chain;
+  double chain_flops = 0;
+  hipStream_t chain_stream = nullptr;
   bool call_split = false;
   int* status = nullptr;
   int* status_host = nullptr;
@@ -318,7 +322,10 @@
 static_assert(kScaleTensors < 63, "the adaptation counter is the last of the 64 words at ut_context::calib");
 constexpr int kCalibHeadroom = 4;
 
+int flush_chain(ut_handle h);
+
 int begin_call(ut_handle h, hipStream_t s) {
+  if (const int rc = flush_chain(h)) return rc;
   h->counter_next = 0;
   ++h->word_gen;
   HIPCHK(h, ut::launch_zero_words(h->counters, 2 * kMaxCounters, s));
@@ -347,9 +354,10 @@
 }
 template <class Launch>
 int bracket_launch(ut_handle h, hipStream_t s, int in_tid, const unsigned* in_max, double flops, int kind, const char* what,
-                   Launch launch) {
+                   Launch launch, int convs = 1) {
+  if (const int rc = flush_chain(h)) return rc;
   if (h->calibrating && in_max && in_tid >= 0 && in_tid < kScaleTensors) HIPCHK(h, ut::launch_merge_max(h->calib + in_tid, in_max, s));
-  ProfEvent pe{nullptr, nullptr, flops, kind};
+  ProfEvent pe{nullptr, nullptr, flops, kind, convs};
   if (h->profiling) {
     HIPCHK(h, hipEventCreateWithFlags(&pe.a, hipEventDisableSystemFence));
     HIPCHK(h, hipEventCreateWithFlags(&pe.b, hipEventDisableSystemFence));
@@ -362,6 +370,19 @@
     h->prof.push_back(pe);
   }
   return UT_OK;
+}
+
+int flush_chain(ut_handle h) {
+  if (h->chain.empty()) return UT_OK;
+  std::vector<ut::ConvLaunch> layers;
+  layers.swap(h->chain);
+  const double flops = h->chain_flops;
+  h->chain_flops = 0;
+  hipStream_t s = h->chain_stream;
+  if (layers.size() == 1)
+    return bracket_launch(h, s, -1, nullptr, flops, 1, "conv_w4", [&] { return ut::launch_conv_w4(layers[0], s); });
+  return bracket_launch(h, s, -1, nullptr, flops, 1, "conv_w4 chain",
+                        [&] { return ut::launch_conv_w4_chain(layers.data(), (int)layers.size(), s); }, (int)layers.size());
 }
 
 int run_conv(ut_handle h, const ConvW& cw, const float* in, const float* res, float* out, int n_img, int H, int W,
@@ -411,7 +432,19 @@
     c.out_max = h->counters + kMaxCounters + word;
     if (out_max) *out_max = c.out_max;
   }
-  return bracket_launch(h, s, kind ? in_tid : -1, in_max, cw.flops_per_pixel * (double)n_img * c.Ho * c.Wo, kind,
+  const double flops = cw.flops_per_pixel * (double)n_img * c.Ho * c.Wo;
+  const ut::W4Form form = kernel == ut::CONV_W4 ? ut::conv_w4_form(c) : ut::W4_NONE;
+  if (kind && (form == ut::W4_TILES128 || form == ut::W4_MAP24) && !(c.no_resident & ut::NO_W4_CHAIN) && h->block_fusion &&
+      !h->calibrating && !h->latency_mode && h->scale_mode == UT_SPLIT_SCALE_CALIBRATED && c.in_max && !c.split_adaptive &&
+      ut::conv_w4_chain_fills(c)) {
+    if (!h->chain.empty() && (h->chain_stream != s || (int)h->chain.size() == ut::W4_MAX_CHAIN || !ut::conv_w4_chainable(h->chain.back(), c)))
+      if ((rc = flush_chain(h))) return rc;
+    h->chain.push_back(c);
+    h->chain_flops += flops;
+    h->chain_stream = s;
+    return UT_OK;
+  }
+  return bracket_launch(h, s, kind ? in_tid : -1, in_max, flops, kind,
                         ut::kConvKernelName[kernel], [&] { return ut::launch_conv_on(kernel, c, s); });
 }
 
@@ -506,7 +539,7 @@
     float t = 0;
     HIPCHK(h, hipEventElapsedTime(&t, pe.a, pe.b));
     const int k = pe.kind ? 1 : 0;
-    ms[k] += t; flops[k] += pe.flops; launches[k] += 1;
+    ms[k] += t; flops[k] += pe.flops; launches[k] += pe.convs;
   }
   prof_clear(h);
   return UT_OK;
@@ -664,6 +697,7 @@
 static int run_stem(ut_handle h, const float* crops, const uint8_t* crops_u8, float* out, int n, hipStream_t st,
                     unsigned** out_max) {
   *out_max = nullptr;
+  if (const int rc = flush_chain(h)) return rc;
   if (h->call_split && !h->latency_mode) {
     const int rc = lease_words(h, st, 1);
     if (rc) return rc;
@@ -674,8 +708,17 @@
   return UT_OK;
 }
 
+static int backbone_pass_launches(ut_handle h, const float* crops, const uint8_t* crops_u8, float* feat, int c0, int n, int off,
+                                  int chunk, hipStream_t s);
 static int backbone_pass(ut_handle h, const float* crops, const uint8_t* crops_u8, float* feat, int c0, int n, int off,
                          int chunk, hipStream_t s) {
+  int rc = backbone_pass_launches(h, crops, crops_u8, feat, c0, n, off, chunk, s);
+  if (!rc) rc = flush_chain(h);
+  if (rc) { h->chain.clear(); h->chain_flops = 0; }
+  return rc;
+}
+static int backbone_pass_launches(ut_handle h, const float* crops, const uint8_t* crops_u8, float* feat, int c0, int n, int off,
+                                  int chunk, hipStream_t s) {
   int rc;
   const size_t a48 = (size_t)off * 48 * 48 * 32, a24 = (size_t)off * 24 * 24 * 64, a12 = (size_t)off * 12 * 12 * 128;
   if ((rc = lease_words(h, s, 256))) return rc;
@@ -694,6 +737,7 @@
       hw = (hw + 2 - 3) / h->bb[b].conv1.stride + 1;
       float* t = x; x = y; y = t;
     }
+    if ((rc = flush_chain(h))) return rc;
     if (done == 0) l2_max = xm;
     else if (l2_max && xm) HIPCHK(h, ut::launch_merge_max(l2_max, xm, s));
     else l2_max = nullptr;
@@ -952,7 +996,8 @@
   rc = run_block(h, blocks[0], b.regin, b.rega, nullptr, b.regb, S, 6, 6, s, in_word, &mid_word, head_split ? tid0 : -1, head_split ? tid0 + 1 : -1);
   if (!rc) rc = run_block(h, blocks[1], b.regb, b.rega, nullptr, b.regin, S, 6, 6, s, mid_word, nullptr, head_split ? tid0 + 2 : -1, head_split ? tid0 + 3 : -1);
   h->call_split = false;
-  if (rc) return rc;
+  if (!rc) rc = flush_chain(h);
+  if (rc) { h->chain.clear(); h->chain_flops = 0; return rc; }
   HIPCHK(h, ut::launch_pool_decode(a, b.regin, reg.c, stride, reg.w_out, reg.b_out, reg.d, out_pose, out_raw, b.rega, s));
   return UT_OK;
 }
@@ -1538,7 +1583,7 @@
 
 int ut_set_resident_weights(ut_handle h, int on) {
   if (!h) return UT_E_INVALID;
-  if (on < 0 || on > 6) return fail(h, UT_E_INVALID, "ut_set_resident_weights: bad argument");
+  if (on < 0 || on > 7) return fail(h, UT_E_INVALID, "ut_set_resident_weights: bad argument");
   h->resident_weights = on;
   return UT_OK;
 }
diff --git a/absolutetrack_amd/csrc/ut_kernels.h b/absolutetrack_amd/csrc/ut_kernels.h
--- a/absolutetrack_amd/csrc/ut_kernels.h
+++ b/absolutetrack_amd/csrc/ut_kernels.h
@@ -83,6 +83,21 @@
 enum W4Form : int { W4_NONE = 0, W4_TILES128, W4_MAP24, W4_STRIDE2 };
 W4Form conv_w4_form(const ConvLaunch& c);
 hipError_t launch_conv_w4(const ConvLaunch& c, hipStream_t s);
+constexpr int W4_MAX_CHAIN = 9;
+struct W4Layer {
+  const float* in; const float* res; float* out; const void* w_split; const float* bias;
+  const unsigned* in_max;
+  unsigned* out_max;
+  float split_unscale;
+  int k_cin, relu;
+};
+struct W4ChainLaunch : ConvLaunch {
+  int n_layers;
+  W4Layer lay[W4_MAX_CHAIN];
+};
+bool conv_w4_chainable(const ConvLaunch& a, const ConvLaunch& b);
+bool conv_w4_chain_fills(const ConvLaunch& c);
+hipError_t launch_conv_w4_chain(const ConvLaunch* layers, int n_layers, hipStream_t s);
 bool conv_c64k_applicable(const ConvLaunch& c);
 hipError_t launch_conv_c64k(const ConvLaunch& c, hipStream_t s);
 struct BlockLaunch {
@@ -122,8 +137,9 @@
   NO_W4 = 2,
   NO_W4_MAP24 = 4,
   NO_W4_STRIDE2 = 8,
-};
-constexpr int kResidentKinds[7] = {
+  NO_W4_CHAIN = 16,
+};
+constexpr int kResidentKinds[8] = {
     NO_C64K | NO_W4 | NO_W4_MAP24 | NO_W4_STRIDE2,
     0,
     NO_W4 | NO_W4_MAP24 | NO_W4_STRIDE2,
@@ -131,6 +147,7 @@
     NO_W4_MAP24 | NO_W4_STRIDE2,
     NO_C64K | NO_W4_MAP24 | NO_W4_STRIDE2,
     NO_W4_STRIDE2,
+    NO_W4_CHAIN,
 };
 
 inline bool conv_prefers_patch(const ConvLaunch& c) {
```

Result: faster. 173,200 hand-frames/s, median of 6 (+2.9%).
